# irfanfadhullah/unet_zoo

Measured on AMD Instinct MI355X. Metric: images/sec (fwd+bwd) at B=16 3x256x256, 1/2/4/8 MI355X, higher is better.
Workload: dtype bf16; 1 GPU; unet train step (zero_grad+fwd+BCE+bwd+clip+AdamW), B=16/GPU 3x256x256, random-init weights; global_batch=16, parallelism=dp1

## Files before the change

include/unetzoo_hip.h:

```cpp
#ifndef UNETZOO_HIP_H
#define UNETZOO_HIP_H

#include <stddef.h>
#include <stdint.h>

#ifdef __cplusplus
extern "C" {
#endif

#define UZ_ABI_VERSION 1

enum { UZ_F32 = 0, UZ_BF16 = 1 };

enum {
  UZ_OK = 0,
  UZ_EINVAL = -1,
  UZ_ENOTIMPL = -2
};

enum {
  UZ_TAPS_CONV = 0,
  UZ_TAPS_GATHER2X2 = 1,
  UZ_TAPS_CONV_UP2 = 2,
  UZ_TAPS_CONV_S2 = 3
// ... 5 lines not shown

int uz_abi_version(void);
const char* uz_last_error_string(void);
int uz_profile_arm(void* start_event, void* stop_event);
int uz_profile_disarm(void);
int uz_build_ablate(void);
const char* uz_source_hash(void);
int uz_clock_probe(int iters, void* out_pairs, int workgroups, void* stream);
int uz_set_cu_reserve(int n);
int uz_get_cu_reserve(void);

typedef struct uz_conv_desc {
  int dtype;
  int N, H, W;
  int Hin, Win;
  int Cin, ldx;
  int Nout, ldy;
  int ntaps, taps_mode, dil;
  int store_mode, Co;
  int Hout, Wout;
} uz_conv_desc;

int uz_conv_igemm_grid_m(const uz_conv_desc* d);
int uz_conv_igemm_kernel_name(const uz_conv_desc* d, int with_workspace, char* buf, int cap);
int uz_conv_igemm(const uz_conv_desc* d, const void* x, const void* w_packed, const float* bias,
                  void* y, float* stats_partial, void* stream);
int uz_conv_igemm_res(const uz_conv_desc* d, const void* x, const void* w_packed, const float* bias,
                      const void* res, int ldres, void* y, void* stream);
int uz_conv_igemm_res_ws(const uz_conv_desc* d, const void* x, const void* w_packed, const float* bias,
                         const void* res, int ldres, void* y, void* workspace, void* stream);
long long uz_conv_igemm_workspace_bytes(const uz_conv_desc* d);
int uz_conv_igemm_ws_grid_m(const uz_conv_desc* d);
int uz_conv_igemm_ws(const uz_conv_desc* d, const void* x, const void* w_packed, const float* bias,
                     void* y, float* stats_partial, void* workspace, void* stream);
int uz_conv_igemm_bnred_supported(const uz_conv_desc* d);
int uz_conv_igemm_bnred(const uz_conv_desc* d, const void* x, const void* w_packed, void* y, const void* bn_y,
                        int ld_bny, const float* scale, const float* shift, const float* mean, const float* invstd,
                        float* partial, void* stream);

int uz_conv_igemm_xf_supported(const uz_conv_desc* d);
int uz_conv_igemm_xf(const uz_conv_desc* d, const void* x, const float* in_scale, const float* in_shift,
                     const void* w_packed, const float* bias, void* y, float* stats_partial, void* stream);

typedef struct uz_wgrad_desc {
  int dtype;
  int N, H, W;
  int Hr, Wr;
  int Ci, ldl;
  int Cj, ldr;
  int ntaps, taps_mode, dil;
} uz_wgrad_desc;

int uz_wgrad_split(const uz_wgrad_desc* d);
long long uz_wgrad_workspace_bytes(const uz_wgrad_desc* d);
int uz_wgrad(const uz_wgrad_desc* d, const void* L, const void* R, float* out, void* workspace,
             void* stream);
int uz_wgrad_kernel_name(const uz_wgrad_desc* d, char* buf, int cap);
int uz_wgrad_xf_supported(const uz_wgrad_desc* d);
int uz_wgrad_xf(const uz_wgrad_desc* d, const void* L, const void* R, const float* r_scale, const float* r_shift,
                float* out, void* workspace, void* stream, int phase);
int uz_wgrad_phase(const uz_wgrad_desc* d, const void* L, const void* R, float* out, void* workspace, void* stream,
                   int phase);
typedef struct {
  uz_wgrad_desc desc;
  const void* L;
  const void* R;
  float* out;
} uz_wgrad_item;
long long uz_wgrad_multi_workspace_bytes(const uz_wgrad_item* items, int n);
int uz_wgrad_multi(const uz_wgrad_item* items, int n, void* workspace, void* stream);
long long uz_wgrad_batched_workspace_bytes(const uz_wgrad_desc* d, int batch);
int uz_wgrad_batched(const uz_wgrad_desc* d, int batch, const void* L, long long lb, const void* R, long long rb,
                     float* out, long long ob, void* workspace, void* stream);
int uz_wgrad_batched2(const uz_wgrad_desc* d, int batch, int batch2, const void* L, long long lb, long long lb2, const void* R,
                      long long rb, long long rb2, float* out, long long ob, void* workspace, void* stream);

int uz_conv3x3_first_supported(int dtype, int C, int Cout);
int uz_conv3x3_first_rows(int N, int H, int W);
int uz_conv3x3_first_fwd(int dtype, const float* x, int N, int C, int H, int W, const float* w, const float* bias, int Cout,
                         void* y, int ldy, float* stats, void* stream);
long long uz_conv3x3_first_wgrad_workspace_bytes(int N, int H, int W, int Cout);
int uz_conv3x3_first_wgrad(int dtype, const float* x, int N, int C, int H, int W, const void* dy, int lddy, int Cout, float* dw,
                           void* workspace, void* stream);

enum { UZ_PACK_CONV_FWD = 0, UZ_PACK_CONV_DGRAD = 1, UZ_PACK_CONVT_FWD = 2, UZ_PACK_CONVT_DGRAD = 3,
       UZ_PACK_IM2COL = 4, UZ_PACK_VEC_REPEAT = 5 };
int uz_pack_weights(int dtype, int mode, const float* w, int Co, int Ci, int T, int Kpad, void* dst,
                    void* stream);
typedef struct uz_pack_item {
  const float* src;
  void* dst;
  long long begin;
  int mode, Co, Ci, T, Kpad;
  int pad_;
} uz_pack_item;
int uz_pack_weights_batched(int dtype, const uz_pack_item* items_device, int n_items,
                            long long total_elements, void* stream);
typedef struct uz_pack3x3_item {
  const float* src;
  void* dst_fwd;
  void* dst_dgrad;
  int Co, Ci;
  int tile_begin;
  int pad_;
} uz_pack3x3_item;
int uz_pack_conv3x3_batched(int dtype, const uz_pack3x3_item* items_device, int n_items, int total_tiles,
                            void* stream);

int uz_im2col3x3_nchw(int dtype, const float* x_nchw, int N, int C, int H, int W, int Kpad, void* dst,
                      void* stream);

int uz_bn_finalize(const float* stats_partial, int grid_m, int C, double count, const float* gamma,
                   const float* beta, float eps, float momentum, float* running_mean,
                   float* running_var, float* scale, float* shift, float* mean, float* invstd,
                   void* stream);
int uz_bn_eval_scale(int C, const float* gamma, const float* beta, const float* running_mean,
                     const float* running_var, float eps, float* scale, float* shift, void* stream);

int uz_bn_relu_apply(int dtype, const void* y, int ldy, const float* scale, const float* shift,
                     int N, int H, int W, int C, void* act, int lda, void* pooled, int ldp,
                     void* stream);
int uz_bn_relu_add_apply(int dtype, const void* y, int ldy, const float* scale, const float* shift,
                         int N, int H, int W, int C, const void* res, int ldr, void* act, int lda,
                         void* pooled, int ldp, int pool_ceil, void* stream);
int uz_bn_relu_add_apply_fin(int dtype, const void* y, int ldy, const float* stats_partial, int rows, double count,
                             const float* gamma, const float* beta, float eps, float momentum, float* running_mean,
                             float* running_var, float* vec, int* flag, int N, int H, int W, int C, const void* res, int ldr,
                             void* act, int lda, void* pooled, int ldp, int pool_ceil, void* stream);

typedef struct uz_bnbwd_desc {
  int dtype;
  int N, H, W, C;
  int ldy, ldg0, ldg1, ldgp, lddy;
  int pool_ceil;
} uz_bnbwd_desc;
int uz_colstats_rows(int dtype, int P, int C);
int uz_colstats(int dtype, const void* x, int ld, int P, int C, float* partial, void* stream);
long long uz_bn_relu_bwd_workspace_bytes(const uz_bnbwd_desc* d, int has_pool_grad);
int uz_bn_relu_bwd_reduce(const uz_bnbwd_desc* d, const void* y, const float* scale,
                          const float* shift, const float* mean, const float* invstd, const void* g0,
                          const void* g1, const void* gpool, void* workspace, double* sums,
                          float* dgamma, float* dbeta, void* stream);
int uz_bn_relu_bwd_apply(const uz_bnbwd_desc* d, const void* y, const float* scale,
                         const float* shift, const float* mean, const float* invstd, const void* g0,
                         const void* g1, const void* gpool, const double* sums, double count,
                         void* dy, void* stream);
int uz_bn_relu_bwd_reduce_rows(const uz_bnbwd_desc* d, const void* y, const float* scale, const float* shift,
                               const float* mean, const float* invstd, const void* g0, const void* g1, const void* gpool,
                               void* workspace, void* stream);
int uz_bn_relu_bwd_apply_fin(const uz_bnbwd_desc* d, const void* y, const float* scale, const float* shift,
                             const float* mean, const float* invstd, const void* g0, const void* g1, const void* gpool,
                             const float* partial, int rows, double* sums, float* dgamma, float* dbeta, int* flag,
                             double count, void* dy, void* stream);
int uz_bn_bwd_finalize(const float* partial, int rows, int C, double* sums, float* dgamma, float* dbeta, void* stream);

int uz_outconv_fwd(int dtype, const void* x, int ldx, int N, int HW, int C, const float* w,
                   const float* b, int Kout, float* out_nchw, void* stream);
int uz_outconv_fwd_xf(int dtype, const void* y, int ldy, int N, int HW, int C, const float* scale, const float* shift,
                      const float* w, const float* b, int Kout, float* out_nchw, void* stream);
long long uz_outconv_bwd_workspace_bytes(int dtype, int N, int HW, int C, int Kout);
int uz_outconv_bwd(int dtype, const void* x, int ldx, int N, int HW, int C, const float* w, int Kout,
                   const float* g_nchw, void* dx, int lddx, float* dw, float* db, void* workspace,
                   void* stream);
int uz_outconv_bwd_rows(int dtype, int N, int HW, int C);
int uz_outconv_bwd_bnred(int dtype, const void* x, int ldx, int N, int HW, int C, const float* w, int Kout,
                         const float* g_nchw, void* dx, int lddx, float* dw, float* db, void* workspace,
                         const void* bn_y, int ld_bny, const float* scale, const float* shift, const float* mean,
                         const float* invstd, float* bn_partial, void* stream);

int uz_attn_grid(int dtype, int P, int channels);
int uz_attn_psi_fwd(int dtype, const void* g1raw, int ldg, const void* x1raw, int ldx, const float* vec_g,
                    const float* vec_x, const float* wpsi, const float* bpsi ,
                    int P, int F, float* q, float* partial , void* stream);
int uz_attn_gate_fwd(int dtype, const void* x, int ldx, const float* q, const float* vec_q, int P, int C,
                     void* out, int ldo, void* stream);
int uz_attn_bwd_psi(int dtype, const void* dout, int ldd, const void* x, int ldx, const float* q,
                    const float* vec_q, int P, int C, void* dx_direct, int lddx, float* dz,
                    float* partial , void* stream);
int uz_attn_bwd_reduce(int dtype, const void* g1raw, int ldg, const void* x1raw, int ldx, const float* q,
                       const float* dz, const float* wpsi, const float* vec_g, const float* vec_x,
                       const float* vec_q, const double* a01, int P, int F,
                       float* partial , void* stream);
int uz_attn_bwd_apply(int dtype, const void* g1raw, int ldg, const void* x1raw, int ldx, const float* q,
                      const float* dz, const float* wpsi, const float* vec_g, const float* vec_x,
                      const float* vec_q, const double* a01, const double* totals, int P, int F,
                      void* dg1raw, int lddg, void* dx1raw, int lddx, void* stream);
int uz_sum_rows(const float* partial, int rows, int n, double* out, void* stream);
int uz_sum_rows_f32(const float* partial, int rows, int n, float* out0, int n0, float* out1, void* stream);
int uz_sum_rows_f32_ld(const float* partial, int ld, int rows, int n, float* out0, int n0, float* out1,
                       void* stream);
int uz_sum2x2(int dtype, const void* du, int ldu, int N, int H, int W, int C, void* dx, int lddx,
              void* stream);

int uz_bilinear_fwd(int dtype, const void* x, int ldx, long long x_img_stride, int N, int Hi, int Wi,
                    int C, void* y, int ldy, long long y_img_stride, int Ho, int Wo, void* stream);
int uz_bilinear_bwd(int dtype, const void* g, int ldg, long long g_img_stride, int N, int Hi, int Wi,
                    int C, void* dx, int lddx, long long dx_img_stride, int Ho, int Wo, void* stream);
int uz_resize_bilinear_fwd(int dtype, const void* x, int ldx, long long x_img_stride, int N, int Hi, int Wi,
                           int C, void* y, int ldy, long long y_img_stride, int Ho, int Wo, int align_corners,
                           void* stream);
int uz_resize_bilinear_bwd(int dtype, const void* g, int ldg, long long g_img_stride, int N, int Hi, int Wi,
                           int C, void* dx, int lddx, long long dx_img_stride, int Ho, int Wo, int align_corners,
                           void* stream);
int uz_resample2(int dtype, const void* src, int lds, int N, int Hs, int Ws, int C, void* dst, int ldd, int Hd,
                 int Wd, int mode, void* stream);
int uz_pool_grad_combine(int dtype, int N, int H, int W, int C, const void* act, int lda, const void* g0,
                         int ldg0, const void* g1, int ldg1, const void* gp, int ldgp, void* out, int ldo,
                         int pool_ceil, void* stream);
int uz_sideconv3x3_fwd(int dtype, const void* x, int ldx, int N, int H, int W, int C, const float* w,
                       const float* bias, float* taps_ws, float* out, long long out_img_stride,
                       void* stream);
long long uz_sideconv3x3_bwd_workspace_bytes(int dtype, int N, int H, int W, int C);
int uz_sideconv3x3_bwd(int dtype, const void* x, int ldx, int N, int H, int W, int C, const float* w,
                       const float* g, long long g_img_stride, void* dx, int lddx, float* dw, float* db,
                       void* workspace, void* stream);
int uz_fuse1x1_fwd(const float* d, int N, int HW, int Cc, int K, const float* w, const float* b,
                   float* out, void* stream);
long long uz_fuse1x1_bwd_workspace_bytes(int N, int HW, int Cc, int K);
int uz_fuse1x1_bwd(const float* d, int N, int HW, int Cc, int K, const float* w, const float* g,
                   const float* const* g_extra, int n_extra, float* dcat, float* dw, float* db,
                   void* workspace, void* stream);

int uz_patchify(int dtype, const float* x_nchw, int N, int C, int H, int W, int patch, int Kpad,
                void* out, void* stream);

enum { UZ_LN_PLAIN = 0, UZ_LN_MERGE = 1, UZ_LN_EXPAND = 2 };
typedef struct uz_ln_desc {
  int dtype, N, Ho, Wo, C;
  int ldx, ldy, ldr, ldg, lddx;
  int mode, r;
  float eps;
  int act;
} uz_ln_desc;
int uz_layernorm_fwd(const uz_ln_desc* d, const void* x, const float* gamma, const float* beta,
                     const void* res, const float* image_scale, void* y, float* stats, void* stream);
int uz_layernorm_bwd_rows(const uz_ln_desc* d);
int uz_layernorm_bwd(const uz_ln_desc* d, const void* x, const float* gamma, const float* stats,
// ... 185 lines not shown
```

unet_zoo_amd/_lib.py:

```python
from __future__ import annotations

import ctypes
import os
from ctypes import POINTER, Structure, c_char_p, c_double, c_float, c_int, c_void_p

import torch

UZ_F32, UZ_BF16 = 0, 1
TAPS_CONV, TAPS_GATHER2X2, TAPS_CONV_UP2, TAPS_CONV_S2 = 0, 1, 2, 3
STORE_PLAIN, STORE_SHUFFLE2X2 = 0, 1
PACK_CONV_FWD, PACK_CONV_DGRAD, PACK_CONVT_FWD, PACK_CONVT_DGRAD, PACK_IM2COL, PACK_VEC_REPEAT = range(6)

LIB_NAME = "libunetzoo_hip.so"
LIB_PATH = os.environ.get("UNET_ZOO_AMD_LIB") or os.path.join(os.path.dirname(os.path.abspath(__file__)), LIB_NAME)

EXPORTS = (
    "uz_abi_version", "uz_last_error_string", "uz_build_ablate", "uz_source_hash", "uz_set_cu_reserve", "uz_get_cu_reserve", "uz_clock_probe", "uz_conv_igemm_grid_m", "uz_conv_igemm",
    "uz_wgrad_split", "uz_wgrad_workspace_bytes", "uz_wgrad", "uz_wgrad_kernel_name", "uz_wgrad_phase", "uz_wgrad_xf_supported", "uz_wgrad_xf", "uz_conv3x3_first_supported", "uz_conv3x3_first_rows", "uz_conv3x3_first_fwd",
    "uz_conv3x3_first_wgrad_workspace_bytes", "uz_conv3x3_first_wgrad", "uz_pack_weights", "uz_pack_weights_batched", "uz_pack_conv3x3_batched", "uz_im2col3x3_nchw", "uz_bn_finalize",
    "uz_bn_eval_scale", "uz_bn_relu_apply", "uz_bn_relu_bwd_workspace_bytes", "uz_bn_relu_bwd_reduce", "uz_bn_relu_bwd_apply",
    "uz_outconv_fwd", "uz_outconv_fwd_xf", "uz_outconv_bwd_workspace_bytes", "uz_outconv_bwd", "uz_outconv_bwd_rows", "uz_outconv_bwd_bnred",
    "uz_colsum",
    "uz_attn_grid", "uz_attn_psi_fwd", "uz_attn_gate_fwd", "uz_attn_bwd_psi", "uz_attn_bwd_reduce",
    "uz_attn_bwd_apply", "uz_sum_rows", "uz_sum_rows_f32", "uz_sum2x2",
    "uz_bn_relu_add_apply", "uz_bn_relu_add_apply_fin", "uz_bn_relu_bwd_reduce_rows", "uz_bn_relu_bwd_apply_fin", "uz_bilinear_fwd", "uz_bilinear_bwd", "uz_resize_bilinear_fwd", "uz_resize_bilinear_bwd", "uz_resample2",
    "uz_pool_grad_combine",
    "uz_sideconv3x3_fwd", "uz_sideconv3x3_bwd_workspace_bytes", "uz_sideconv3x3_bwd",
    "uz_fuse1x1_fwd", "uz_fuse1x1_bwd_workspace_bytes", "uz_fuse1x1_bwd",
    "uz_conv_igemm_workspace_bytes", "uz_conv_igemm_ws_grid_m", "uz_conv_igemm_ws",
    "uz_conv_igemm_bnred_supported", "uz_conv_igemm_bnred", "uz_conv_igemm_xf_supported", "uz_conv_igemm_xf", "uz_conv_igemm_kernel_name", "uz_bn_bwd_finalize", "uz_profile_arm", "uz_profile_disarm",
    "uz_patchify", "uz_layernorm_fwd", "uz_layernorm_bwd_rows", "uz_layernorm_bwd", "uz_layernorm_act_bwd",
    "uz_ln_head_fwd", "uz_ln_head_bwd_workspace_bytes", "uz_ln_head_bwd", "uz_sum_rows_f32_ld",
    "uz_winattn_fwd", "uz_winattn_bwd_rows", "uz_winattn_bwd",
    "uz_colsum_workspace_bytes", "uz_colsum_ws", "uz_colstats_rows", "uz_colstats", "uz_cpb_fwd", "uz_cpb_bwd",
    "uz_cpb_fwd_batched", "uz_cpb_bwd_batched_workspace_bytes", "uz_cpb_bwd_batched",
    "uz_clip_adamw_workspace_bytes", "uz_clip_adamw",
    "uz_gelu_fwd", "uz_gelu_bwd", "uz_dwconv3x3", "uz_dwconv3x3_wgrad_rows", "uz_dwconv3x3_wgrad",
    "uz_space_to_depth", "uz_space_to_depth_crop", "uz_im2col_nchw", "uz_sra_fwd", "uz_sra_bwd_workspace_bytes", "uz_sra_bwd",
    "uz_bce_dice_workspace_bytes", "uz_bce_dice", "uz_colsum_batched_workspace_bytes", "uz_colsum_batched", "uz_sum_rows_f32_batched", "uz_conv_igemm_res", "uz_wgrad_multi_workspace_bytes", "uz_wgrad_multi", "uz_conv_igemm_res_ws",
    "uz_add_relu", "uz_relu_bwd", "uz_pil_resample_h_u8", "uz_pil_resample_v_f32",
    "uz_gemm_nt", "uz_softmax_fwd", "uz_softmax_bwd", "uz_adaptive_avgpool_fwd", "uz_adaptive_avgpool_bwd",
    "uz_rowdot_f32", "uz_cast_rows", "uz_wgrad_batched_workspace_bytes", "uz_wgrad_batched", "uz_wgrad_batched2",
    "uz_softmax_workspace_bytes", "uz_add_map", "uz_dropout", "uz_chanscale_relu", "uz_chanattn_probs_fwd", "uz_chanattn_probs_bwd",
    "uz_conv5x5_grid_m", "uz_conv5x5", "uz_wgrad5x5_workspace_bytes", "uz_wgrad5x5",
    "uz_bn_elu_apply", "uz_bn_elu_bwd_rows", "uz_bn_elu_bwd_reduce", "uz_bn_elu_bwd_apply",
)


class ConvDesc(Structure):
    _fields_ = [(n, c_int) for n in (
        "dtype", "N", "H", "W", "Hin", "Win", "Cin", "ldx", "Nout", "ldy", "ntaps", "taps_mode",
        "dil", "store_mode", "Co", "Hout", "Wout")]


class WgradDesc(Structure):
    _fields_ = [(n, c_int) for n in (
        "dtype", "N", "H", "W", "Hr", "Wr", "Ci", "ldl", "Cj", "ldr", "ntaps", "taps_mode", "dil")]


class Conv5Desc(Structure):
    _fields_ = [(n, c_int) for n in ("dtype", "N", "H", "W", "Cin", "ldx", "Nout", "ldy", "ksize")]


class Wgrad5Desc(Structure):
    _fields_ = [(n, c_int) for n in ("dtype", "N", "H", "W", "Ci", "ldl", "Cj", "ldr", "ksize", "CiOut", "CjOut")]


class BnEluBwdDesc(Structure):
    _fields_ = [(n, c_int) for n in ("dtype", "N", "HW", "C", "ldx", "ldo", "ldg0", "ldg1", "ldg2", "lddx", "ldgres", "flags")]


class BnBwdDesc(Structure):
    _fields_ = [(n, c_int) for n in (
        "dtype", "N", "H", "W", "C", "ldy", "ldg0", "ldg1", "ldgp", "lddy", "pool_ceil")]


class LnDesc(Structure):
    _fields_ = [(n, c_int) for n in ("dtype", "N", "Ho", "Wo", "C", "ldx", "ldy", "ldr", "ldg", "lddx", "mode", "r")] \
        + [("eps", c_float), ("act", c_int)]


class WinAttnDesc(Structure):
    _fields_ = [(n, c_int) for n in ("dtype", "B", "H", "W", "C", "heads", "ws", "shift", "Nt", "ldq", "ldo")] \
        + [("scale", c_float)]


class SraDesc(Structure):
    _fields_ = [(n, c_int) for n in ("dtype", "B", "N", "NK", "heads", "head_dim", "kps", "ldq", "ldk", "ldv", "ldo")] \
        + [("scale", c_float)]


class GemmDesc(Structure):
    _fields_ = [(n, c_int) for n in ("dtype", "batch", "M", "N", "K", "ldx", "ldw", "ldy", "ldres")] \
        + [(n, ctypes.c_longlong) for n in ("xb", "wb", "yb", "resb")] + [("batch2", c_int)] \
        + [(n, ctypes.c_longlong) for n in ("xb2", "wb2", "yb2", "resb2")]


class WgradItem(Structure):
    _fields_ = [("desc", WgradDesc), ("L", c_void_p), ("R", c_void_p), ("out", c_void_p)]


class SumRowsItem(Structure):
    _fields_ = [("partial", c_void_p), ("out0", c_void_p), ("out1", c_void_p), ("rows", c_int), ("n", c_int), ("n0", c_int),
                ("reserved", c_int)]
# ... 16 lines not shown
    _fields_ = [("src", c_void_p), ("dst", c_void_p), ("begin", ctypes.c_longlong), ("mode", c_int),
                ("Co", c_int), ("Ci", c_int), ("T", c_int), ("Kpad", c_int), ("pad_", c_int)]


class Pack3x3Item(Structure):
    _fields_ = [("src", c_void_p), ("dst_fwd", c_void_p), ("dst_dgrad", c_void_p), ("Co", c_int), ("Ci", c_int),
                ("tile_begin", c_int), ("pad_", c_int)]


class HipLibraryError(RuntimeError):
    pass


_lib = None


def load():
    global _lib
    if _lib is not None:
        return _lib
    if not os.path.exists(LIB_PATH):
        raise HipLibraryError(
            f"{LIB_PATH} not found: the HIP kernel library is not built. Run "
            "`python -c 'import __graft_entry__ as g; g.build()'` from the repo root. "
            "unet_zoo_amd has no CPU fallback.")
    lib = ctypes.CDLL(LIB_PATH)
    lib.uz_abi_version.restype = c_int
    lib.uz_last_error_string.restype = c_char_p
    lib.uz_source_hash.restype = c_char_p
    lib.uz_source_hash.argtypes = []
    vp, ip, fp = c_void_p, c_int, c_float
    lib.uz_set_cu_reserve.argtypes = [c_int]
    lib.uz_clock_probe.argtypes = [c_int, vp, c_int, vp]
    lib.uz_get_cu_reserve.argtypes = []
    lib.uz_conv_igemm_grid_m.argtypes = [POINTER(ConvDesc)]
    lib.uz_conv_igemm.argtypes = [POINTER(ConvDesc), vp, vp, vp, vp, vp, vp]
    lib.uz_conv_igemm_res.argtypes = [POINTER(ConvDesc), vp, vp, vp, vp, ip, vp, vp]
    lib.uz_conv_igemm_res_ws.argtypes = [POINTER(ConvDesc), vp, vp, vp, vp, ip, vp, vp, vp]
    lib.uz_conv_igemm_workspace_bytes.argtypes = [POINTER(ConvDesc)]
    lib.uz_conv_igemm_ws_grid_m.argtypes = [POINTER(ConvDesc)]
    lib.uz_conv_igemm_ws.argtypes = [POINTER(ConvDesc), vp, vp, vp, vp, vp, vp, vp]
    lib.uz_conv_igemm_bnred_supported.argtypes = [POINTER(ConvDesc)]
    lib.uz_conv_igemm_xf_supported.argtypes = [POINTER(ConvDesc)]
    lib.uz_conv_igemm_xf.argtypes = [POINTER(ConvDesc), vp, vp, vp, vp, vp, vp, vp, vp]
    lib.uz_conv_igemm_kernel_name.argtypes = [POINTER(ConvDesc), c_int, c_char_p, c_int]
    lib.uz_profile_arm.argtypes = [vp, vp]
    lib.uz_profile_disarm.argtypes = []
    lib.uz_conv_igemm_bnred.argtypes = [POINTER(ConvDesc), vp, vp, vp, vp, c_int, vp, vp, vp, vp, vp, vp]
    lib.uz_bn_bwd_finalize.argtypes = [vp, c_int, c_int, vp, vp, vp, vp]
    lib.uz_patchify.argtypes = [ip, vp, ip, ip, ip, ip, ip, ip, vp, vp]
    lib.uz_layernorm_fwd.argtypes = [POINTER(LnDesc), vp, vp, vp, vp, vp, vp, vp, vp]
    lib.uz_layernorm_act_bwd.argtypes = [POINTER(LnDesc), vp, vp, vp, vp, vp, vp, vp, vp]
    lib.uz_layernorm_bwd_rows.argtypes = [POINTER(LnDesc)]
    lib.uz_layernorm_bwd.argtypes = [POINTER(LnDesc), vp, vp, vp, vp, vp, vp, vp, vp]
    lib.uz_ln_head_fwd.argtypes = [POINTER(LnDesc), vp, vp, vp, vp, vp, ip, vp, vp, vp]
    lib.uz_ln_head_bwd_workspace_bytes.argtypes = [POINTER(LnDesc), ip]
    lib.uz_ln_head_bwd.argtypes = [POINTER(LnDesc), vp, vp, vp, vp, ip, vp, vp, vp, vp, vp, vp, vp, vp, vp]
    lib.uz_sum_rows_f32_ld.argtypes = [vp, ip, ip, ip, vp, ip, vp, vp]
    lib.uz_winattn_fwd.argtypes = [POINTER(WinAttnDesc), vp, vp, vp, vp, vp, vp]
    lib.uz_winattn_bwd_rows.argtypes = [POINTER(WinAttnDesc)]
    lib.uz_winattn_bwd.argtypes = [POINTER(WinAttnDesc), vp, vp, vp, vp, vp, vp, ip, vp, ip, vp, vp]
    lib.uz_colstats_rows.argtypes = [ip, ip, ip]
    lib.uz_colstats.argtypes = [ip, vp, ip, ip, ip, vp, vp]
    lib.uz_cpb_fwd.argtypes = [vp, vp, vp, vp, vp, ip, ip, ip, vp, vp]
    lib.uz_cpb_bwd.argtypes = [vp, vp, vp, vp, vp, ip, ip, ip, vp, vp, vp, vp, vp]
    lib.uz_cpb_fwd_batched.argtypes = [vp, ip, vp]
    lib.uz_cpb_bwd_batched_workspace_bytes.argtypes = [vp, ip]
    lib.uz_cpb_bwd_batched.argtypes = [vp, ip, vp, vp]
    lib.uz_clip_adamw_workspace_bytes.argtypes = []
    lib.uz_clip_adamw.argtypes = [vp, vp, vp, vp, ctypes.c_longlong, fp, fp, fp, fp, fp, fp, vp, vp, vp]
    lib.uz_wgrad_split.argtypes = [POINTER(WgradDesc)]
    lib.uz_wgrad_workspace_bytes.argtypes = [POINTER(WgradDesc)]
    lib.uz_wgrad.argtypes = [POINTER(WgradDesc), vp, vp, vp, vp, vp]
    lib.uz_wgrad_kernel_name.argtypes = [POINTER(WgradDesc), c_char_p, c_int]
    lib.uz_wgrad_phase.argtypes = [POINTER(WgradDesc), vp, vp, vp, vp, vp, c_int]
    lib.uz_wgrad_xf_supported.argtypes = [POINTER(WgradDesc)]
    lib.uz_wgrad_xf.argtypes = [POINTER(WgradDesc), vp, vp, vp, vp, vp, vp, vp, c_int]
    lib.uz_conv3x3_first_supported.argtypes = [ip, ip, ip]
    lib.uz_conv3x3_first_rows.argtypes = [ip, ip, ip]
    lib.uz_conv3x3_first_fwd.argtypes = [ip, vp, ip, ip, ip, ip, vp, vp, ip, vp, ip, vp, vp]
    lib.uz_conv3x3_first_wgrad_workspace_bytes.argtypes = [ip, ip, ip, ip]
    lib.uz_conv3x3_first_wgrad_workspace_bytes.restype = ctypes.c_longlong
    lib.uz_conv3x3_first_wgrad.argtypes = [ip, vp, ip, ip, ip, ip, vp, ip, ip, vp, vp, vp]
    lib.uz_pack_weights.argtypes = [ip, ip, vp, ip, ip, ip, ip, vp, vp]
    lib.uz_pack_weights_batched.argtypes = [ip, vp, ip, ctypes.c_longlong, vp]
    lib.uz_pack_conv3x3_batched.argtypes = [ip, vp, ip, ip, vp]
    lib.uz_im2col3x3_nchw.argtypes = [ip, vp, ip, ip, ip, ip, ip, vp, vp]
    lib.uz_bn_finalize.argtypes = [vp, ip, ip, c_double, vp, vp, fp, fp, vp, vp, vp, vp, vp, vp, vp]
    lib.uz_bn_eval_scale.argtypes = [ip, vp, vp, vp, vp, fp, vp, vp, vp]
    lib.uz_bn_relu_apply.argtypes = [ip, vp, ip, vp, vp, ip, ip, ip, ip, vp, ip, vp, ip, vp]
    lib.uz_bn_relu_bwd_workspace_bytes.argtypes = [POINTER(BnBwdDesc), ip]
    lib.uz_bn_relu_bwd_reduce.argtypes = [POINTER(BnBwdDesc), vp, vp, vp, vp, vp, vp, vp, vp, vp, vp,
                                          vp, vp, vp]
    lib.uz_bn_relu_bwd_apply.argtypes = [POINTER(BnBwdDesc), vp, vp, vp, vp, vp, vp, vp, vp, vp,
                                         c_double, vp, vp]
    lib.uz_outconv_fwd.argtypes = [ip, vp, ip, ip, ip, ip, vp, vp, ip, vp, vp]
    lib.uz_outconv_fwd_xf.argtypes = [ip, vp, ip, ip, ip, ip, vp, vp, vp, vp, ip, vp, vp]
    lib.uz_outconv_bwd_workspace_bytes.argtypes = [ip, ip, ip, ip, ip]
    lib.uz_outconv_bwd.argtypes = [ip, vp, ip, ip, ip, ip, vp, ip, vp, vp, ip, vp, vp, vp, vp]
    lib.uz_outconv_bwd_rows.argtypes = [ip, ip, ip, ip]
    lib.uz_outconv_bwd_bnred.argtypes = [ip, vp, ip, ip, ip, ip, vp, ip, vp, vp, ip, vp, vp, vp, vp, ip, vp, vp, vp, vp, vp, vp]
    lib.uz_colsum.argtypes = [ip, vp, ip, ip, ip, vp, vp]
    lib.uz_colsum_workspace_bytes.argtypes = [ip, ip, ip]
    lib.uz_colsum_ws.argtypes = [ip, vp, ip, ip, ip, vp, vp, vp]
    lib.uz_attn_grid.argtypes = [ip, ip, ip]
    lib.uz_attn_psi_fwd.argtypes = [ip, vp, ip, vp, ip, vp, vp, vp, vp, ip, ip, vp, vp, vp]
    lib.uz_attn_gate_fwd.argtypes = [ip, vp, ip, vp, vp, ip, ip, vp, ip, vp]
    lib.uz_attn_bwd_psi.argtypes = [ip, vp, ip, vp, ip, vp, vp, ip, ip, vp, ip, vp, vp, vp]
    lib.uz_attn_bwd_reduce.argtypes = [ip, vp, ip, vp, ip, vp, vp, vp, vp, vp, vp, vp, ip, ip, vp, vp]
    lib.uz_attn_bwd_apply.argtypes = [ip, vp, ip, vp, ip, vp, vp, vp, vp, vp, vp, vp, vp, ip, ip, vp, ip,
                                      vp, ip, vp]
    lib.uz_sum_rows.argtypes = [vp, ip, ip, vp, vp]
    lib.uz_sum_rows_f32.argtypes = [vp, ip, ip, vp, ip, vp, vp]
    lib.uz_sum2x2.argtypes = [ip, vp, ip, ip, ip, ip, ip, vp, ip, vp]
    ll = ctypes.c_longlong
    lib.uz_bn_relu_add_apply.argtypes = [ip, vp, ip, vp, vp, ip, ip, ip, ip, vp, ip, vp, ip, vp, ip, ip, vp]
    lib.uz_bn_relu_add_apply_fin.argtypes = [ip, vp, ip, vp, ip, ctypes.c_double, vp, vp, c_float, c_float, vp, vp, vp, vp,
                                             ip, ip, ip, ip, vp, ip, vp, ip, vp, ip, ip, vp]
    lib.uz_bn_relu_bwd_reduce_rows.argtypes = [POINTER(BnBwdDesc), vp, vp, vp, vp, vp, vp, vp, vp, vp, vp]
    lib.uz_bn_relu_bwd_apply_fin.argtypes = [POINTER(BnBwdDesc), vp, vp, vp, vp, vp, vp, vp, vp, vp, ip, vp, vp, vp, vp,
                                             ctypes.c_double, vp, vp]
    lib.uz_bilinear_fwd.argtypes = [ip, vp, ip, ll, ip, ip, ip, ip, vp, ip, ll, ip, ip, vp]
    lib.uz_bilinear_bwd.argtypes = [ip, vp, ip, ll, ip, ip, ip, ip, vp, ip, ll, ip, ip, vp]
    lib.uz_resize_bilinear_fwd.argtypes = [ip, vp, ip, ll, ip, ip, ip, ip, vp, ip, ll, ip, ip, ip, vp]
    lib.uz_resize_bilinear_bwd.argtypes = [ip, vp, ip, ll, ip, ip, ip, ip, vp, ip, ll, ip, ip, ip, vp]
    lib.uz_resample2.argtypes = [ip, vp, ip, ip, ip, ip, ip, vp, ip, ip, ip, ip, vp]
    lib.uz_pool_grad_combine.argtypes = [ip, ip, ip, ip, ip, vp, ip, vp, ip, vp, ip, vp, ip, vp, ip, ip, vp]
    lib.uz_sideconv3x3_fwd.argtypes = [ip, vp, ip, ip, ip, ip, ip, vp, vp, vp, vp, ll, vp]
    lib.uz_sideconv3x3_bwd_workspace_bytes.argtypes = [ip, ip, ip, ip, ip]
    lib.uz_sideconv3x3_bwd.argtypes = [ip, vp, ip, ip, ip, ip, ip, vp, vp, ll, vp, ip, vp, vp, vp, vp]
    lib.uz_fuse1x1_fwd.argtypes = [vp, ip, ip, ip, ip, vp, vp, vp, vp]
    lib.uz_fuse1x1_bwd_workspace_bytes.argtypes = [ip, ip, ip, ip]
    lib.uz_fuse1x1_bwd.argtypes = [vp, ip, ip, ip, ip, vp, vp, POINTER(c_void_p), ip, vp, vp, vp, vp, vp]
    lib.uz_sum_rows_f32_batched.argtypes = [POINTER(SumRowsItem), ip, vp]
    lib.uz_wgrad_multi_workspace_bytes.argtypes = [POINTER(WgradItem), ip]
    lib.uz_wgrad_multi_workspace_bytes.restype = ctypes.c_longlong
    lib.uz_wgrad_multi.argtypes = [POINTER(WgradItem), ip, vp, vp]
    lib.uz_colsum_batched_workspace_bytes.argtypes = [ip, POINTER(ColsumItem), ip]
    lib.uz_colsum_batched.argtypes = [ip, POINTER(ColsumItem), ip, vp, vp]
    lib.uz_bce_dice_workspace_bytes.argtypes = [ll]
    lib.uz_bce_dice.argtypes = [vp, vp, ll, vp, vp, vp, vp]
    lib.uz_gelu_fwd.argtypes = [ip, vp, ip, vp, ip, ll, ip, vp]
    lib.uz_gelu_bwd.argtypes = [ip, vp, ip, vp, ip, vp, ip, ll, ip, vp]
    lib.uz_dwconv3x3.argtypes = [ip, vp, ip, vp, vp, vp, ip, ip, ip, ip, ip, ip, vp]
    lib.uz_dwconv3x3_wgrad_rows.argtypes = [ip, ip, ip, ip, ip]
    lib.uz_dwconv3x3_wgrad.argtypes = [ip, vp, ip, vp, ip, vp, ip, ip, ip, ip, vp]
    lib.uz_space_to_depth.argtypes = [ip, vp, ip, vp, ip, ip, ip, ip, ip, ip, ip, vp]
    lib.uz_space_to_depth_crop.argtypes = [ip, vp, ip, vp, ip, ip, ip, ip, ip, ip, ip, vp]
    lib.uz_im2col_nchw.argtypes = [ip, vp, ip, ip, ip, ip, ip, ip, ip, ip, vp, vp]
    lib.uz_sra_fwd.argtypes = [POINTER(SraDesc), vp, vp, vp, vp, vp, vp]
    lib.uz_sra_bwd_workspace_bytes.argtypes = [POINTER(SraDesc)]
    lib.uz_sra_bwd.argtypes = [POINTER(SraDesc), vp, vp, vp, vp, vp, vp, ip, vp, ip, vp, ip, vp, vp]
    lib.uz_add_relu.argtypes = [ip, vp, ip, vp, ip, vp, ip, ll, ip, vp]
    lib.uz_relu_bwd.argtypes = [ip, vp, ip, vp, ip, vp, ip, ll, ip, vp]
    lib.uz_pil_resample_h_u8.argtypes = [vp, ip, ip, ip, vp, vp, ip, ip, vp, vp]
    lib.uz_pil_resample_v_f32.argtypes = [vp, ip, ip, ip, vp, vp, ip, ip, POINTER(c_float), POINTER(c_float), ip, vp, vp]
    lib.uz_wgrad_batched_workspace_bytes.argtypes = [POINTER(WgradDesc), ip]
    lib.uz_wgrad_batched.argtypes = [POINTER(WgradDesc), ip, vp, ll, vp, ll, vp, ll, vp, vp]
    lib.uz_wgrad_batched2.argtypes = [POINTER(WgradDesc), ip, ip, vp, ll, ll, vp, ll, ll, vp, ll, vp, vp]
    lib.uz_gemm_nt.argtypes = [POINTER(GemmDesc), vp, vp, vp, vp, vp, vp]
    lib.uz_softmax_workspace_bytes.argtypes = [ip, ip, ip, ip]
    lib.uz_softmax_fwd.argtypes = [ip, vp, ip, ll, ip, ip, ip, ip, c_float, vp, vp]
    lib.uz_chanattn_probs_fwd.argtypes = [ip, vp, ip, ip, ip, ip, c_float, c_float, vp, vp, vp]
    lib.uz_chanattn_probs_bwd.argtypes = [ip, vp, vp, ip, ip, ip, ip, c_float, c_float, vp, vp, vp]
    lib.uz_dropout.argtypes = [ip, vp, ip, vp, c_float, vp, ip, ll, ip, vp]
    lib.uz_chanscale_relu.argtypes = [ip, ip, vp, ip, vp, ip, vp, vp, ip, ip, ip, vp, ip, vp]
    lib.uz_add_map.argtypes = [ip, vp, ip, vp, vp, ip, ll, ip, ip, vp]
    lib.uz_softmax_bwd.argtypes = [ip, vp, vp, ip, ll, ip, ip, ip, ip, c_float, vp, ip, vp]
    lib.uz_adaptive_avgpool_fwd.argtypes = [ip, vp, ip, ip, ip, ip, ip, vp, ip, ip, ip, vp]
    lib.uz_adaptive_avgpool_bwd.argtypes = [ip, vp, ip, ip, ip, ip, ip, vp, ip, ip, ip, ip, vp]
    lib.uz_rowdot_f32.argtypes = [ip, vp, ip, vp, ip, ll, ip, vp, vp]
    lib.uz_cast_rows.argtypes = [ip, vp, ip, vp, ip, ll, ip, ip, vp]
    lib.uz_conv5x5_grid_m.argtypes = [POINTER(Conv5Desc)]
    lib.uz_conv5x5.argtypes = [POINTER(Conv5Desc), vp, vp, vp, vp, vp, vp]
    lib.uz_wgrad5x5_workspace_bytes.argtypes = [POINTER(Wgrad5Desc)]
    lib.uz_wgrad5x5.argtypes = [POINTER(Wgrad5Desc), vp, vp, vp, vp, vp]
    lib.uz_bn_elu_apply.argtypes = [ip, vp, ip, vp, vp, ip, ip, ip, vp, ip, vp, ip, vp, ip, vp, ip, vp]
    lib.uz_bn_elu_bwd_rows.argtypes = [POINTER(BnEluBwdDesc)]
    lib.uz_bn_elu_bwd_reduce.argtypes = [POINTER(BnEluBwdDesc), vp, vp, vp, vp, vp, vp, vp, vp, vp, vp, vp, vp]
    lib.uz_bn_elu_bwd_apply.argtypes = [POINTER(BnEluBwdDesc), vp, vp, vp, vp, vp, vp, vp, vp, vp, vp, vp, vp, vp, vp]
    for name in EXPORTS:
        fn = getattr(lib, name)
        if name not in ("uz_last_error_string", "uz_source_hash"):
# ... 74 lines not shown
```

unet_zoo_amd/csrc/uz_conv_first.hip:

```cpp
#include "uz_common.h"

namespace {

constexpr int TH = 8, TW = 32, PH = TH + 2, PW = TW + 2;
constexpr int STG = 144;

struct CfArgs {
  const float* x;
  const float* w;
  const float* bias;
  void* y;
  float* stats;
  const void* dy;
  float* slab;
  int N, C, H, W, Cout, ldy, th_n, tw_n, ntiles;
};

__device__ __forceinline__ float round_bf16(float v) { return (float)(bf16_t)v; }

__device__ __forceinline__ unsigned halo_fetch(const CfArgs& a, float (&h)[4], int tile, int tid) {
  const int per = a.th_n * a.tw_n;
  const int img = tile / per, rem = tile - img * per;
  const int h0 = (rem / a.tw_n) * TH, w0 = (rem % a.tw_n) * TW;
  const int n = a.C * PH * PW;
  unsigned mask = 0;
#pragma unroll
  for (int j = 0; j < 4; ++j) {
    const int idx = tid + 256 * j;
    const int c = idx / (PH * PW), r2 = idx - c * (PH * PW);
    const int r = r2 / PW, col = r2 - r * PW;
    const int gh = h0 - 1 + r, gw = w0 - 1 + col;
    const bool ok = idx < n && (unsigned)gh < (unsigned)a.H && (unsigned)gw < (unsigned)a.W;
    h[j] = a.x[ok ? (((size_t)img * a.C + c) * a.H + gh) * a.W + gw : 0];
    mask |= ok ? 1u << j : 0u;
  }
  return mask;
}
__device__ __forceinline__ void halo_store(float* sx, const float (&h)[4], unsigned mask, int tid, int n) {
#pragma unroll
  for (int j = 0; j < 4; ++j)
    if (tid + 256 * j < n) sx[tid + 256 * j] = (mask >> j & 1u) ? round_bf16(h[j]) : 0.f;
}
static_assert(3 * PH * PW <= 4 * 256, "four halo elements per thread");

template <int CT>
__global__ __launch_bounds__(256) void conv_first_fwd_kernel(const CfArgs a) {
  __shared__ float sx[3 * PH * PW];
  __shared__ __attribute__((aligned(16))) float sbias[64];
  __shared__ __attribute__((aligned(16))) char sstg[4][32 * STG];
  __shared__ float sred[4][2][CT * 32];
  const int tid = threadIdx.x, lane = tid & 63, wave = tid >> 6;
  const int px = lane & 31, b = lane >> 5;
  const int per = a.th_n * a.tw_n;
  const int K = a.C * 9;
  float hreg[4];
  unsigned hmask = 0;
  if ((int)blockIdx.x < a.ntiles) hmask = halo_fetch(a, hreg, blockIdx.x, tid);
  if (tid < 64) sbias[tid] = (a.bias != nullptr && tid < a.Cout) ? a.bias[tid] : 0.f;

  bf16x8 wfr[CT][2];
  float wraw[CT][2][8];
#pragma unroll
  for (int t = 0; t < CT; ++t)
#pragma unroll
    for (int kh = 0; kh < 2; ++kh)
#pragma unroll
      for (int i = 0; i < 8; ++i) {
        const int k = 16 * kh + 8 * b + i, co = 32 * t + px;
        wraw[t][kh][i] = a.w[(k < K && co < a.Cout) ? (size_t)co * K + k : 0];
      }
#pragma unroll
  for (int t = 0; t < CT; ++t)
#pragma unroll
    for (int kh = 0; kh < 2; ++kh)
#pragma unroll
      for (int i = 0; i < 8; ++i) asm volatile("" : "+v"(wraw[t][kh][i]));
#pragma unroll
  for (int t = 0; t < CT; ++t)
#pragma unroll
    for (int kh = 0; kh < 2; ++kh)
#pragma unroll
      for (int i = 0; i < 8; ++i) {
        const int k = 16 * kh + 8 * b + i, co = 32 * t + px;
        wfr[t][kh][i] = (bf16_t)((k < K && co < a.Cout) ? wraw[t][kh][i] : 0.f);
      }
  int koff[2][8];
#pragma unroll
  for (int kh = 0; kh < 2; ++kh)
#pragma unroll
    for (int i = 0; i < 8; ++i) {
      const int k = 16 * kh + 8 * b + i;
      const int c = k / 9, t9 = k - c * 9, ty = t9 / 3, tx = t9 - ty * 3;
      koff[kh][i] = (k < K ? (c * PH + ty) * PW + tx : 0) + px;
    }
  constexpr int CPP = CT * 4;
  constexpr int PPI = 64 / CPP;
  const int ch = lane % CPP;
  float st1[8], st2[8];
// ... 1 lines not shown
  for (int e = 0; e < 8; ++e) st1[e] = st2[e] = 0.f;

  char* stg = sstg[wave];
  bf16_t* yg = static_cast<bf16_t*>(a.y);
#pragma unroll 1
  for (int tile = blockIdx.x; tile < a.ntiles; tile += gridDim.x) {
    const int img = tile / per, rem = tile - img * per;
    const int h0 = (rem / a.tw_n) * TH, w0 = (rem % a.tw_n) * TW;
    __syncthreads();
    halo_store(sx, hreg, hmask, tid, a.C * PH * PW);
    __syncthreads();
    {
      const int nxt = tile + (int)gridDim.x;
      hmask = halo_fetch(a, hreg, nxt < a.ntiles ? nxt : tile, tid);
    }
#pragma unroll
    for (int rr = 0; rr < 2; ++rr) {
      const int row = 2 * wave + rr, gh = h0 + row;
      bf16x8 pfr[2];
#pragma unroll
      for (int kh = 0; kh < 2; ++kh)
#pragma unroll
        for (int i = 0; i < 8; ++i) pfr[kh][i] = (bf16_t)sx[koff[kh][i] + row * PW];
#pragma unroll
      for (int t = 0; t < CT; ++t) {
        f32x16 acc;
#pragma unroll
        for (int r = 0; r < 16; ++r) acc[r] = 0.f;
        acc = __builtin_amdgcn_mfma_f32_32x32x16_bf16(wfr[t][0], pfr[0], acc, 0, 0, 0);
        acc = __builtin_amdgcn_mfma_f32_32x32x16_bf16(wfr[t][1], pfr[1], acc, 0, 0, 0);
#pragma unroll
        for (int g4 = 0; g4 < 4; ++g4) {
          const f32x4 bq = *reinterpret_cast<const f32x4*>(sbias + 32 * t + 8 * g4 + 4 * b);
          bf16x4 o;
#pragma unroll
          for (int e = 0; e < 4; ++e) o[e] = (bf16_t)(acc[4 * g4 + e] + bq[e]);
          *reinterpret_cast<bf16x4*>(stg + px * STG + (32 * t + 8 * g4 + 4 * b) * 2) = o;
        }
      }
      __builtin_amdgcn_wave_barrier();
#pragma unroll
      for (int j = 0; j < 32 / PPI; ++j) {
        const int p = j * PPI + lane / CPP;
        const bf16x8 v = *reinterpret_cast<const bf16x8*>(stg + p * STG + ch * 16);
        const int gw = w0 + p;
        if (gh < a.H && gw < a.W && ch * 8 < a.Cout) {
          *reinterpret_cast<bf16x8*>(yg + (((size_t)img * a.H + gh) * a.W + gw) * a.ldy + ch * 8) = v;
#pragma unroll
          for (int e = 0; e < 8; ++e) {
            const float f = (float)v[e];
            st1[e] += f;
            st2[e] += f * f;
          }
        }
      }
      __builtin_amdgcn_wave_barrier();
    }
  }
  if (a.stats == nullptr) return;
  __syncthreads();
  float* red = reinterpret_cast<float*>(sstg[wave]);
#pragma unroll
  for (int e = 0; e < 8; ++e) {
    red[lane * 16 + e] = st1[e];
    red[lane * 16 + 8 + e] = st2[e];
  }
  __builtin_amdgcn_wave_barrier();
#pragma unroll
  for (int idx = lane; idx < CPP * 16; idx += 64) {
    const int c2 = idx / 16, v2 = idx % 16;
    float sacc = 0.f;
#pragma unroll
    for (int q = 0; q < PPI; ++q) sacc += red[(q * CPP + c2) * 16 + v2];
    sred[wave][v2 >> 3][c2 * 8 + (v2 & 7)] = sacc;
  }
  __syncthreads();
  if (tid < 2 * CT * 32) {
    const int q = tid / (CT * 32), co = tid % (CT * 32);
    const float sum = (sred[0][q][co] + sred[1][q][co]) + (sred[2][q][co] + sred[3][q][co]);
    if (co < a.Cout) a.stats[((size_t)blockIdx.x * 2 + q) * a.Cout + co] = sum;
  }
}

template <int CT>
__global__ __launch_bounds__(256) void conv_first_wgrad_kernel(const CfArgs a) {
  constexpr int RB = CT * 64;
  __shared__ float sx[3 * PH * PW];
  __shared__ __attribute__((aligned(16))) char sdy[TH * TW * RB];
  static_assert(4 * CT * 16 * 64 * 4 == TH * TW * RB, "the waves' accumulators meet in the dy tile's LDS");
  float (*sacc)[CT][16][64] = reinterpret_cast<float (*)[CT][16][64]>(sdy);
  const int tid = threadIdx.x, lane = tid & 63, wave = tid >> 6;
  const int l31 = lane & 31, b = lane >> 5;
  const int per = a.th_n * a.tw_n;
  const int K = a.C * 9;
  const bf16_t* dyg = static_cast<const bf16_t*>(a.dy);

  const int k = l31;
  const int kc = k / 9, kt = k - kc * 9, kty = kt / 3, ktx = kt - kty * 3;
  const int pbase = (k < K) ? (kc * PH + kty) * PW + ktx + 8 * b : 0;
  const int g = lane >> 4, q4 = (lane & 15) >> 2, p4 = lane & 3;
  const int lk = 8 * (g >> 1) + q4, lcol = 16 * (g & 1) + 4 * p4;
  typedef __attribute__((address_space(3))) bf16x4* lds_bf16x4_ptr;

  f32x16 acc[CT];
#pragma unroll
  for (int t = 0; t < CT; ++t)
#pragma unroll
    for (int r = 0; r < 16; ++r) acc[t][r] = 0.f;

  constexpr int CPP = RB / 16;
  constexpr int NDY = TH * TW * CPP / 256;
  float hreg[4];
  f32x4 dreg[NDY];
  unsigned hmask = 0, dmask = 0;
  auto dy_fetch = [&](int tile) __attribute__((always_inline)) {
    const int img = tile / per, rem = tile - img * per;
    const int h0 = (rem / a.tw_n) * TH, w0 = (rem % a.tw_n) * TW;
#pragma unroll
    for (int j = 0; j < NDY; ++j) {
      const int idx = tid + 256 * j;
      const int p = idx / CPP, ch = idx % CPP;
      const int r = p / TW, c = p % TW, gh = h0 + r, gw = w0 + c;
      const bool ok = gh < a.H && gw < a.W && ch * 8 < a.Cout;
      dreg[j] = *reinterpret_cast<const f32x4*>(ok ? dyg + (((size_t)img * a.H + gh) * a.W + gw) * a.ldy + ch * 8 : dyg);
      dmask |= ok ? 1u << j : 0u;
    }
  };
  if ((int)blockIdx.x < a.ntiles) {
    hmask = halo_fetch(a, hreg, blockIdx.x, tid);
    dy_fetch(blockIdx.x);
  }
#pragma unroll 1
  for (int tile = blockIdx.x; tile < a.ntiles; tile += gridDim.x) {
    __syncthreads();
    halo_store(sx, hreg, hmask, tid, a.C * PH * PW);
#pragma unroll
    for (int j = 0; j < NDY; ++j) {
      const int idx = tid + 256 * j;
      const int p = idx / CPP, ch = idx % CPP;
      const int gran = ch >> 2, sw = (p >> 1) & 1;
      const int pg = (CT == 2) ? (gran ^ sw) : gran;
      const f32x4 z4 = {0.f, 0.f, 0.f, 0.f};
      *reinterpret_cast<f32x4*>(sdy + p * RB + pg * 64 + (ch & 3) * 16) = (dmask >> j & 1u) ? dreg[j] : z4;
    }
    __syncthreads();
    {
      const int nxt = tile + (int)gridDim.x, ft = nxt < a.ntiles ? nxt : tile;
      hmask = halo_fetch(a, hreg, ft, tid);
      dmask = 0;
      dy_fetch(ft);
    }
#pragma unroll
    for (int rr = 0; rr < 2; ++rr)
#pragma unroll
      for (int half = 0; half < 2; ++half) {
        const int row = 2 * wave + rr, c0 = 16 * half;
        bf16x8 pfr;
#pragma unroll
        for (int i = 0; i < 8; ++i) pfr[i] = (bf16_t)sx[pbase + row * PW + c0 + i];
#pragma unroll
        for (int t = 0; t < CT; ++t) {
          const int p = row * TW + c0 + lk;
          const int sw = (p >> 1) & 1;
          const int gr = (CT == 2) ? (t ^ sw) : 0;
          const char* ad = sdy + p * RB + gr * 64 + lcol * 2;
          const bf16x4 lo = __builtin_amdgcn_ds_read_tr16_b64_v4bf16((lds_bf16x4_ptr)(ad));
          const bf16x4 hi = __builtin_amdgcn_ds_read_tr16_b64_v4bf16((lds_bf16x4_ptr)(ad + 4 * RB));
          const bf16x8 dfr = __builtin_shufflevector(lo, hi, 0, 1, 2, 3, 4, 5, 6, 7);
          acc[t] = __builtin_amdgcn_mfma_f32_32x32x16_bf16(dfr, pfr, acc[t], 0, 0, 0);
        }
      }
  }
  __syncthreads();
#pragma unroll
  for (int t = 0; t < CT; ++t)
#pragma unroll
    for (int r = 0; r < 16; ++r) sacc[wave][t][r][lane] = acc[t][r];
  __syncthreads();
  for (int idx = tid; idx < CT * 16 * 64; idx += 256) {
    const int t = idx / (16 * 64), r = (idx / 64) % 16, l = idx % 64;
    const float s = (sacc[0][t][r][l] + sacc[1][t][r][l]) + (sacc[2][t][r][l] + sacc[3][t][r][l]);
    const int co = 32 * t + (r & 3) + 8 * (r >> 2) + 4 * (l >> 5), kk = l & 31;
    if (co < a.Cout) a.slab[((size_t)blockIdx.x * a.Cout + co) * 32 + kk] = s;
  }
}

__global__ __launch_bounds__(256) void conv_first_wgrad_reduce_kernel(const float* __restrict__ slab, int nwg, int Cout, int K,
                                                                     float* __restrict__ dw) {
  __shared__ float part[16][17];
  const int o = threadIdx.x & 15, zg = threadIdx.x >> 4;
  const int idx = blockIdx.x * 16 + o;
  const size_t stride = (size_t)Cout * 32;
  float s = 0.f;
  int z = zg;
  for (; z + 7 * 16 < nwg; z += 8 * 16) {
    float v[8];
#pragma unroll
    for (int u = 0; u < 8; ++u) v[u] = slab[(size_t)(z + 16 * u) * stride + idx];
#pragma unroll
    for (int u = 0; u < 8; ++u) s += v[u];
  }
  for (; z < nwg; z += 16) s += slab[(size_t)z * stride + idx];
  part[zg][o] = s;
  __syncthreads();
  if (zg == 0) {
    float t = 0.f;
#pragma unroll
    for (int q = 0; q < 16; ++q) t += part[q][o];
    const int co = idx >> 5, k = idx & 31;
    if (k < K) dw[(size_t)co * K + k] = t;
  }
}

int check(int dtype, int N, int C, int H, int W, int Cout, int ld, const char* what) {
  UZ_REQUIRE(dtype == UZ_BF16, "%s: bf16 only (the fp32 run mode takes the im2col path)", what);
  UZ_REQUIRE(N > 0 && H > 0 && W > 0 && C >= 1 && C <= 3, "%s: C = %d not in 1 .. 3", what, C);
  UZ_REQUIRE((Cout == 32 || Cout == 64) && ld >= Cout && ld % 8 == 0, "%s: Cout = %d (32 or 64), ld = %d", what, Cout, ld);
  UZ_REQUIRE((long long)N * H * W * ld * 2 < (1LL << 40), "%s: too large", what);
  return UZ_OK;
}

void fill(CfArgs& a, int N, int C, int H, int W, int Cout, int ld) {
  a.N = N;
  a.C = C;
  a.H = H;
  a.W = W;
  a.Cout = Cout;
  a.ldy = ld;
  a.th_n = (H + TH - 1) / TH;
  a.tw_n = (W + TW - 1) / TW;
  a.ntiles = N * a.th_n * a.tw_n;
}

}

extern "C" int uz_conv3x3_first_supported(int dtype, int C, int Cout) {
  return dtype == UZ_BF16 && C >= 1 && C <= 3 && (Cout == 32 || Cout == 64);
}

static int first_fwd_grid(int ntiles) {
  const int cap = 3 * UZ_NUM_CU_HW;
  return ntiles < cap ? ntiles : cap;
}

extern "C" int uz_conv3x3_first_rows(int N, int H, int W) {
  return first_fwd_grid(N * ((H + TH - 1) / TH) * ((W + TW - 1) / TW));
}

extern "C" int uz_conv3x3_first_fwd(int dtype, const float* x, int N, int C, int H, int W, const float* w, const float* bias,
                                    int Cout, void* y, int ldy, float* stats, void* stream) {
  const int rc = check(dtype, N, C, H, W, Cout, ldy, "uz_conv3x3_first_fwd");
  if (rc != UZ_OK) return rc;
  UZ_REQUIRE(x && w && y && ((uintptr_t)y & 15) == 0, "uz_conv3x3_first_fwd: null / unaligned pointer");
  CfArgs a = {};
  a.x = x;
  a.w = w;
  a.bias = bias;
  a.y = y;
  a.stats = stats;
  fill(a, N, C, H, W, Cout, ldy);
  hipStream_t s = static_cast<hipStream_t>(stream);
  const int grid = first_fwd_grid(a.ntiles);
  if (Cout == 64) hipLaunchKernelGGL(conv_first_fwd_kernel<2>, dim3(grid), dim3(256), 0, s, a);
  else hipLaunchKernelGGL(conv_first_fwd_kernel<1>, dim3(grid), dim3(256), 0, s, a);
  UZ_LAUNCH_CHECK("uz_conv3x3_first_fwd");
  return UZ_OK;
}

static int first_wgrad_grid(int ntiles) {
  const int cap = 3 * UZ_NUM_CU_HW;
  return ntiles < cap ? ntiles : cap;
}

extern "C" long long uz_conv3x3_first_wgrad_workspace_bytes(int N, int H, int W, int Cout) {
  const int ntiles = N * ((H + TH - 1) / TH) * ((W + TW - 1) / TW);
  return (long long)first_wgrad_grid(ntiles) * Cout * 32 * (long long)sizeof(float);
}

extern "C" int uz_conv3x3_first_wgrad(int dtype, const float* x, int N, int C, int H, int W, const void* dy, int lddy,
                                      int Cout, float* dw, void* workspace, void* stream) {
  const int rc = check(dtype, N, C, H, W, Cout, lddy, "uz_conv3x3_first_wgrad");
  if (rc != UZ_OK) return rc;
  UZ_REQUIRE(x && dy && dw && workspace && ((uintptr_t)dy & 15) == 0, "uz_conv3x3_first_wgrad: null / unaligned pointer");
  CfArgs a = {};
  a.x = x;
  a.dy = dy;
  a.slab = static_cast<float*>(workspace);
  fill(a, N, C, H, W, Cout, lddy);
  const int grid = first_wgrad_grid(a.ntiles);
  hipStream_t s = static_cast<hipStream_t>(stream);
  if (Cout == 64) hipLaunchKernelGGL(conv_first_wgrad_kernel<2>, dim3(grid), dim3(256), 0, s, a);
  else hipLaunchKernelGGL(conv_first_wgrad_kernel<1>, dim3(grid), dim3(256), 0, s, a);
  UZ_LAUNCH_CHECK("uz_conv3x3_first_wgrad");
  hipLaunchKernelGGL(conv_first_wgrad_reduce_kernel, dim3(Cout * 32 / 16), dim3(256), 0, s, a.slab, grid, Cout, C * 9, dw);
  UZ_LAUNCH_CHECK("uz_conv3x3_first_wgrad(reduce)");
  return UZ_OK;
}
```

unet_zoo_amd/csrc/uz_eltwise.hip:

```cpp
#include "uz_common.h"

namespace {

template <typename T> __device__ __forceinline__ void load_f(const T* p, float* f) {
  const Vec16<T> v = ld16(p);
#pragma unroll
  for (int i = 0; i < ElemTraits<T>::VEC; ++i) f[i] = (float)v.v[i];
}
template <typename T> __device__ __forceinline__ void store_f(T* p, const float* f) {
  Vec16<T> v;
#pragma unroll
  for (int i = 0; i < ElemTraits<T>::VEC; ++i) v.v[i] = (T)f[i];
  st16(p, v);
}

template <int EW>
__global__ __launch_bounds__(1024) void bn_finalize_kernel(
    const float* __restrict__ part, int grid_m, int C, double count, const float* __restrict__ gamma,
    const float* __restrict__ beta, float eps, float momentum, float* running_mean,
    float* running_var, float* scale, float* shift, float* mean, float* invstd) {
  constexpr int NG = 1024 / EW;
  __shared__ double sh[2][NG][EW + 1];
  const int cl = threadIdx.x % EW, g = threadIdx.x / EW;
  const int c = blockIdx.x * EW + cl;
// ... 414 lines not shown
        for (int i = 0; i < VEC; ++i) yv[k][i] = gv[k][i] = 0.f;
        continue;
      }
      load_f(y + p * a.ldy + c0, yv[k]);
      if (g0 != nullptr) {
        load_f(g0 + p * a.ldg0 + c0, gv[k]);
      } else {
#pragma unroll
        for (int i = 0; i < VEC; ++i) gv[k][i] = 0.f;
      }
      if (g1 != nullptr) {
        float t[VEC];
        load_f(g1 + p * a.ldg1 + c0, t);
#pragma unroll
        for (int i = 0; i < VEC; ++i) gv[k][i] += t[i];
      }
    }
#endif
    if constexpr (POOL) {
      if (gp != nullptr && has_pool) {
        float gpv[VEC];
#ifndef UZ_BN_BRANCHY
#pragma unroll
        for (int i = 0; i < VEC; ++i) gpv[i] = (float)gpr.v[i];
#else
        load_f(gp + gpoff + c0, gpv);
#endif
#pragma unroll
        for (int i = 0; i < VEC; ++i) {
          float best = fmaf(yv[0][i], sc[i], sh[i]);
          if (!norelu) best = fmaxf(best, 0.f);
          int bk = 0;
#pragma unroll
          for (int k = 1; k < 4; ++k) {
            float v = fmaf(yv[k][i], sc[i], sh[i]);
            if (!norelu) v = fmaxf(v, 0.f);
            if (in[k] && v > best) {
              best = v;
              bk = k;
            }
          }
#pragma unroll
          for (int k = 0; k < 4; ++k) gv[k][i] += (k == bk) ? gpv[i] : 0.f;
        }
      }
    }
#pragma unroll
    for (int k = 0; k < NPIX; ++k) {
      if (!in[k]) continue;
      float out[VEC];
#pragma unroll
      for (int i = 0; i < VEC; ++i) {
        const float pre = fmaf(yv[k][i], sc[i], sh[i]);
        const float dz = (norelu || pre > 0.f) ? gv[k][i] : 0.f;
        const float xh = (yv[k][i] - mu[i]) * is[i];
        if (PASS == 1) {
          S0[i] += dz;
          S1[i] += dz * xh;
        } else {
          out[i] = sc[i] * (dz - k0[i] - xh * k1[i]);
        }
      }
      if (PASS == 2) {
        store_f(dy + pix[k] * a.lddy + c0, out);
      }
    }
  }

  if (PASS == 1) {
    float* mine = red + ((size_t)threadIdx.y * blockDim.x + threadIdx.x) * (2 * VEC);
#pragma unroll
    for (int i = 0; i < VEC; ++i) {
      mine[i] = S0[i];
      mine[VEC + i] = S1[i];
    }
    __syncthreads();
    for (int e = threadIdx.y; e < 2 * VEC; e += blockDim.y) {
      float t = 0.f;
      for (int r = 0; r < (int)blockDim.y; ++r) t += red[((size_t)r * blockDim.x + threadIdx.x) * (2 * VEC) + e];
      if (cok) {
        const int which = e / VEC, ch = c0 + (e % VEC);
        a.partials[((size_t)blockIdx.x * 2 + which) * a.C + ch] = t;
      }
    }
  }
}

template <int EW>
__global__ __launch_bounds__(1024) void bn_bwd_finalize_kernel(const float* __restrict__ part, int rows,
                                                               int C, double* __restrict__ sums,
                                                               float* dgamma, float* dbeta) {
  constexpr int NG = 1024 / EW;
  __shared__ double sh[2][NG][EW + 1];
  const int cl = threadIdx.x % EW, g = threadIdx.x / EW;
  const int c = blockIdx.x * EW + cl;
  double a1 = 0.0, a2 = 0.0;
  const int cq = c < C ? c : 0;
  for (int r = g; r < rows; r += 4 * NG) {
    float p1[4], p2[4];
#pragma unroll
    for (int k = 0; k < 4; ++k) {
      const int rr = r + k * NG < rows ? r + k * NG : 0;
      p1[k] = part[((size_t)rr * 2 + 0) * C + cq];
      p2[k] = part[((size_t)rr * 2 + 1) * C + cq];
    }
#pragma unroll
    for (int k = 0; k < 4; ++k) asm volatile("" : "+v"(p1[k]), "+v"(p2[k]));
#pragma unroll
    for (int k = 0; k < 4; ++k)
      if (r + k * NG < rows && c < C) {
        a1 += (double)p1[k];
        a2 += (double)p2[k];
      }
  }
  sh[0][g][cl] = a1;
  sh[1][g][cl] = a2;
  __syncthreads();
#pragma unroll
  for (int st = NG / 2; st > 0; st >>= 1) {
    if (g < st) {
      sh[0][g][cl] += sh[0][g + st][cl];
      sh[1][g][cl] += sh[1][g + st][cl];
    }
    __syncthreads();
  }
  if (g == 0 && c < C) {
    const double t1 = sh[0][0][cl], t2 = sh[1][0][cl];
    sums[c] = t1;
    sums[C + c] = t2;
    if (dgamma != nullptr) {
      dbeta[c] = (float)t1;
      dgamma[c] = (float)t2;
    }
  }
}

constexpr int OUTCONV_MAXK = 8;
__host__ __device__ inline int lanes_per_pixel(int chunks) {
  int l = 1;
  while (l < chunks) l <<= 1;
  return l;
}

template <typename T, int KOUT, bool XF = false>
__global__ __launch_bounds__(256) void outconv_fwd_kernel(const T* __restrict__ x, int ldx, int N,
                                                          int HW, int C, const float* __restrict__ w,
                                                          const float* __restrict__ b,
                                                          float* __restrict__ out,
                                                          const float* __restrict__ xf_scale = nullptr,
                                                          const float* __restrict__ xf_shift = nullptr) {
  constexpr int VEC = ElemTraits<T>::VEC;
  const int LPP = lanes_per_pixel(C / VEC);
  const int ppb = blockDim.x / LPP;
  const int sub = threadIdx.x % LPP, pl = threadIdx.x / LPP;
  const bool live = sub < C / VEC;
  const int P = N * HW;
  float wr[KOUT][VEC];
#pragma unroll
  for (int k = 0; k < KOUT; ++k)
#pragma unroll
    for (int i = 0; i < VEC; ++i) wr[k][i] = live ? w[k * C + sub * VEC + i] : 0.f;
  float xsc[VEC], xsh[VEC];
  if constexpr (XF) {
#pragma unroll
    for (int i = 0; i < VEC; ++i) {
      xsc[i] = live ? xf_scale[sub * VEC + i] : 0.f;
// ... 815 lines not shown
  BnBwdArgs a = bnbwd_args(d, y, scale, shift, mean, invstd, g0, g1, gpool);
  a.partials = static_cast<float*>(workspace);
  hipStream_t s = (hipStream_t)stream;
  const int rc2 = d->dtype == UZ_BF16 ? bnbwd_launch<bf16_t, 1>(d, a, gpool != nullptr, s)
                                      : bnbwd_launch<float, 1>(d, a, gpool != nullptr, s);
  if (rc2 != UZ_OK) return rc2;
  dim3 grid, block;
  bnbwd_shape(d, gpool != nullptr, &grid, &block);
  bnbwd_finalize(static_cast<const float*>(workspace), (int)grid.x, d->C, sums, dgamma, dbeta, s);
  UZ_LAUNCH_CHECK("uz_bn_relu_bwd_reduce(finalize)");
  return UZ_OK;
}

extern "C" int uz_bn_bwd_finalize(const float* partial, int rows, int C, double* sums, float* dgamma, float* dbeta,
                                  void* stream) {
  UZ_REQUIRE(partial && sums && rows > 0 && C > 0, "uz_bn_bwd_finalize: bad arguments");
  UZ_REQUIRE((dgamma == nullptr) == (dbeta == nullptr), "uz_bn_bwd_finalize: dgamma/dbeta");
  bnbwd_finalize(partial, rows, C, sums, dgamma, dbeta, (hipStream_t)stream);
  UZ_LAUNCH_CHECK("uz_bn_bwd_finalize");
  return UZ_OK;
}

extern "C" int uz_bn_relu_bwd_apply(const uz_bnbwd_desc* d, const void* y, const float* scale,
                                    const float* shift, const float* mean, const float* invstd,
                                    const void* g0, const void* g1, const void* gpool, const double* sums,
                                    double count, void* dy, void* stream) {
  const int rc = bnbwd_check(d, g0, g1, gpool);
  if (rc != UZ_OK) return rc;
  UZ_REQUIRE(y && scale && shift && mean && invstd && sums && dy, "uz_bn_relu_bwd_apply: null pointer");
  UZ_REQUIRE(count > 0, "uz_bn_relu_bwd_apply: count");
  const int vec = d->dtype == UZ_BF16 ? 8 : 4;
  UZ_REQUIRE(d->lddy % vec == 0 && d->lddy >= d->C, "uz_bn_relu_bwd_apply: bad lddy");
  BnBwdArgs a = bnbwd_args(d, y, scale, shift, mean, invstd, g0, g1, gpool);
  a.sums = const_cast<double*>(sums);
  a.dy = dy;
  a.inv_count = 1.0 / count;
  hipStream_t s = (hipStream_t)stream;
  return d->dtype == UZ_BF16 ? bnbwd_launch<bf16_t, 2>(d, a, gpool != nullptr, s)
                             : bnbwd_launch<float, 2>(d, a, gpool != nullptr, s);
}

extern "C" int uz_bn_relu_bwd_reduce_rows(const uz_bnbwd_desc* d, const void* y, const float* scale, const float* shift,
                                          const float* mean, const float* invstd, const void* g0, const void* g1,
                                          const void* gpool, void* workspace, void* stream) {
  const int rc = bnbwd_check(d, g0, g1, gpool);
  if (rc != UZ_OK) return rc;
  UZ_REQUIRE(y && scale && shift && mean && invstd && workspace, "uz_bn_relu_bwd_reduce_rows: null pointer");
  BnBwdArgs a = bnbwd_args(d, y, scale, shift, mean, invstd, g0, g1, gpool);
  a.partials = static_cast<float*>(workspace);
  hipStream_t s = (hipStream_t)stream;
  return d->dtype == UZ_BF16 ? bnbwd_launch<bf16_t, 1>(d, a, gpool != nullptr, s) : bnbwd_launch<float, 1>(d, a, gpool != nullptr, s);
}

extern "C" int uz_bn_relu_bwd_apply_fin(const uz_bnbwd_desc* d, const void* y, const float* scale, const float* shift,
                                        const float* mean, const float* invstd, const void* g0, const void* g1,
                                        const void* gpool, const float* partial, int rows, double* sums, float* dgamma,
                                        float* dbeta, int* flag, double count, void* dy, void* stream) {
  const int rc = bnbwd_check(d, g0, g1, gpool);
  if (rc != UZ_OK) return rc;
  UZ_REQUIRE(y && scale && shift && mean && invstd && sums && dy && partial && flag, "uz_bn_relu_bwd_apply_fin: null pointer");
  UZ_REQUIRE(count > 0 && rows > 0, "uz_bn_relu_bwd_apply_fin: count / rows");
  UZ_REQUIRE((dgamma == nullptr) == (dbeta == nullptr), "uz_bn_relu_bwd_apply_fin: dgamma/dbeta");
  const int vec = d->dtype == UZ_BF16 ? 8 : 4;
  UZ_REQUIRE(d->lddy % vec == 0 && d->lddy >= d->C, "uz_bn_relu_bwd_apply_fin: bad lddy");
  BnBwdArgs a = bnbwd_args(d, y, scale, shift, mean, invstd, g0, g1, gpool);
  a.sums = sums;
  a.dy = dy;
  a.inv_count = 1.0 / count;
  a.fin.part = partial; a.fin.rows = rows; a.fin.ew = fin_ew(rows, d->C);
  a.fin.sums = sums; a.fin.dgamma = dgamma; a.fin.dbeta = dbeta; a.fin.flag = flag;
  hipStream_t s = (hipStream_t)stream;
  dim3 grid, block;
  bnbwd_shape(d, gpool != nullptr, &grid, &block, 2);
  if ((long long)grid.x * grid.y < (d->C + a.fin.ew - 1) / a.fin.ew) {
    bnbwd_finalize(partial, rows, d->C, sums, dgamma, dbeta, s);
    UZ_LAUNCH_CHECK("uz_bn_relu_bwd_apply_fin(finalize)");
    a.fin = BnFin{};
    return d->dtype == UZ_BF16 ? bnbwd_launch<bf16_t, 2>(d, a, gpool != nullptr, s) : bnbwd_launch<float, 2>(d, a, gpool != nullptr, s);
  }
  return d->dtype == UZ_BF16 ? bnbwd_launch<bf16_t, 2, true>(d, a, gpool != nullptr, s)
                             : bnbwd_launch<float, 2, true>(d, a, gpool != nullptr, s);
}

extern "C" int uz_outconv_fwd(int dtype, const void* x, int ldx, int N, int HW, int C, const float* w,
                              const float* b, int Kout, float* out_nchw, void* stream) {
  UZ_REQUIRE(dtype == UZ_F32 || dtype == UZ_BF16, "uz_outconv_fwd: bad dtype");
  const int vec = dtype == UZ_BF16 ? 8 : 4;
  UZ_REQUIRE(x && w && b && out_nchw, "uz_outconv_fwd: null pointer");
  UZ_REQUIRE(Kout >= 1 && Kout <= OUTCONV_MAXK, "uz_outconv_fwd: Kout=%d (max %d)", Kout, OUTCONV_MAXK);
  UZ_REQUIRE(C % vec == 0 && C / vec <= 64, "uz_outconv_fwd: C=%d unsupported", C);
  UZ_REQUIRE(ldx % vec == 0 && ldx >= C && N > 0 && HW > 0 && (long long)N * HW < (1LL << 31),
             "uz_outconv_fwd: bad shape");
  const int ppb = 256 / lanes_per_pixel(C / vec);
  const int grid = grid_for(((long long)N * HW + ppb - 1) / ppb, 1);
  hipStream_t s = (hipStream_t)stream;
  if (dtype == UZ_BF16) {
    UZ_KOUT_SWITCH(Kout, hipLaunchKernelGGL((outconv_fwd_kernel<bf16_t, KOUT>), dim3(grid), dim3(256), 0, s, (const bf16_t*)x, ldx, N, HW, C, w, b, out_nchw, (const float*)nullptr, (const float*)nullptr))
  } else {
    UZ_KOUT_SWITCH(Kout, hipLaunchKernelGGL((outconv_fwd_kernel<float, KOUT>), dim3(grid), dim3(256), 0, s, (const float*)x, ldx, N, HW, C, w, b, out_nchw, (const float*)nullptr, (const float*)nullptr))
  }
  UZ_LAUNCH_CHECK("uz_outconv_fwd");
  return UZ_OK;
}

extern "C" int uz_outconv_fwd_xf(int dtype, const void* y, int ldy, int N, int HW, int C, const float* scale,
                                 const float* shift, const float* w, const float* b, int Kout, float* out_nchw,
                                 void* stream) {
  UZ_REQUIRE(dtype == UZ_BF16, "uz_outconv_fwd_xf: bf16 only");
  UZ_REQUIRE(y && scale && shift && w && b && out_nchw, "uz_outconv_fwd_xf: null pointer");
  UZ_REQUIRE(Kout >= 1 && Kout <= OUTCONV_MAXK, "uz_outconv_fwd_xf: Kout=%d (max %d)", Kout, OUTCONV_MAXK);
  UZ_REQUIRE(C % 8 == 0 && C / 8 <= 64, "uz_outconv_fwd_xf: C=%d unsupported", C);
  UZ_REQUIRE(ldy % 8 == 0 && ldy >= C && N > 0 && HW > 0 && (long long)N * HW < (1LL << 31), "uz_outconv_fwd_xf: bad shape");
  const int ppb = 256 / lanes_per_pixel(C / 8);
  const int grid = grid_for(((long long)N * HW + ppb - 1) / ppb, 1);
  hipStream_t s = (hipStream_t)stream;
  UZ_KOUT_SWITCH(Kout, hipLaunchKernelGGL((outconv_fwd_kernel<bf16_t, KOUT, true>), dim3(grid), dim3(256), 0, s, (const bf16_t*)y, ldy, N, HW, C, w, b, out_nchw, scale, shift))
  UZ_LAUNCH_CHECK("uz_outconv_fwd_xf");
  return UZ_OK;
}

static int outconv_bwd_grid(int dtype, int N, int HW, int C) {
  const int vec = dtype == UZ_BF16 ? 8 : 4;
  const int ppb = 256 / lanes_per_pixel(C / vec);
  long long g = ((long long)N * HW + (long long)ppb * 4 - 1) / ((long long)ppb * 4);
  if (g > UZ_NUM_CU * 4) g = UZ_NUM_CU * 4;
  if (g < 1) g = 1;
  return (int)g;
}

extern "C" long long uz_outconv_bwd_workspace_bytes(int dtype, int N, int HW, int C, int Kout) {
  UZ_REQUIRE(dtype == UZ_F32 || dtype == UZ_BF16, "uz_outconv_bwd_workspace_bytes: bad dtype");
  const int vec = dtype == UZ_BF16 ? 8 : 4;
  UZ_REQUIRE(N > 0 && HW > 0 && Kout >= 1 && Kout <= OUTCONV_MAXK && C % vec == 0 && C / vec <= 64,
             "uz_outconv_bwd_workspace_bytes: bad shape");
  return (long long)outconv_bwd_grid(dtype, N, HW, C) * Kout * (C + 1) * (long long)sizeof(float);
}

extern "C" int uz_outconv_bwd_rows(int dtype, int N, int HW, int C) {
  UZ_REQUIRE(dtype == UZ_F32 || dtype == UZ_BF16, "uz_outconv_bwd_rows: bad dtype");
  return outconv_bwd_grid(dtype, N, HW, C);
}

extern "C" int uz_outconv_bwd_bnred(int dtype, const void* x, int ldx, int N, int HW, int C, const float* w,
                                    int Kout, const float* g_nchw, void* dx, int lddx, float* dw, float* db,
                                    void* workspace, const void* bn_y, int ld_bny, const float* scale,
                                    const float* shift, const float* mean, const float* invstd, float* bn_partial,
                                    void* stream) {
  UZ_REQUIRE(dtype == UZ_BF16, "uz_outconv_bwd_bnred: bf16 only");
  UZ_REQUIRE(w && g_nchw && dw && db && workspace && dx && bn_y && scale && shift && mean && invstd && bn_partial,
             "uz_outconv_bwd_bnred: null pointer");
  UZ_REQUIRE(Kout >= 1 && Kout <= OUTCONV_MAXK, "uz_outconv_bwd_bnred: Kout=%d", Kout);
  UZ_REQUIRE(C % 8 == 0 && C / 8 <= 64, "uz_outconv_bwd_bnred: C=%d unsupported", C);
  UZ_REQUIRE((x == nullptr || (ldx % 8 == 0 && ldx >= C)) && lddx % 8 == 0 && lddx >= C && ld_bny % 8 == 0 && ld_bny >= C && N > 0 &&
                 HW > 0 && (long long)N * HW < (1LL << 31), "uz_outconv_bwd_bnred: bad shape");
  const int g = outconv_bwd_grid(dtype, N, HW, C);
  float* part = static_cast<float*>(workspace);
  hipStream_t s = (hipStream_t)stream;
  if (x != nullptr) {
    UZ_KOUT_SWITCH(Kout, hipLaunchKernelGGL((outconv_bwd_kernel<bf16_t, KOUT, true>), dim3((unsigned)g), dim3(256), 0, s,
                                            (const bf16_t*)x, ldx, N, HW, C, w, g_nchw, (bf16_t*)dx, lddx, part,
                                            (const bf16_t*)bn_y, ld_bny, scale, shift, mean, invstd, bn_partial))
  } else {
    UZ_KOUT_SWITCH(Kout, hipLaunchKernelGGL((outconv_bwd_kernel<bf16_t, KOUT, true, true>), dim3((unsigned)g), dim3(256), 0, s,
                                            (const bf16_t*)nullptr, 0, N, HW, C, w, g_nchw, (bf16_t*)dx, lddx, part,
                                            (const bf16_t*)bn_y, ld_bny, scale, shift, mean, invstd, bn_partial))
  }
  UZ_LAUNCH_CHECK("uz_outconv_bwd_bnred");
  const int ne = Kout * (C + 1);
  hipLaunchKernelGGL(outconv_bwd_finalize_kernel, dim3(uz_cdiv(ne, 32)), dim3(1024), 0, s, part, g, Kout, C, dw, db);
  UZ_LAUNCH_CHECK("uz_outconv_bwd_bnred(finalize)");
  return UZ_OK;
}

extern "C" int uz_outconv_bwd(int dtype, const void* x, int ldx, int N, int HW, int C, const float* w,
                              int Kout, const float* g_nchw, void* dx, int lddx, float* dw, float* db,
                              void* workspace, void* stream) {
  UZ_REQUIRE(dtype == UZ_F32 || dtype == UZ_BF16, "uz_outconv_bwd: bad dtype");
  const int vec = dtype == UZ_BF16 ? 8 : 4;
  UZ_REQUIRE(x && w && g_nchw && dw && db && workspace, "uz_outconv_bwd: null pointer");
  UZ_REQUIRE(Kout >= 1 && Kout <= OUTCONV_MAXK, "uz_outconv_bwd: Kout=%d", Kout);
  UZ_REQUIRE(C % vec == 0 && C / vec <= 64, "uz_outconv_bwd: C=%d unsupported", C);
  UZ_REQUIRE(ldx % vec == 0 && ldx >= C && N > 0 && HW > 0 && (long long)N * HW < (1LL << 31),
             "uz_outconv_bwd: bad shape");
  if (dx) UZ_REQUIRE(lddx % vec == 0 && lddx >= C, "uz_outconv_bwd: bad lddx");
  const int g = outconv_bwd_grid(dtype, N, HW, C);
  float* part = static_cast<float*>(workspace);
  hipStream_t s = (hipStream_t)stream;
  if (dtype == UZ_BF16) {
    UZ_KOUT_SWITCH(Kout, hipLaunchKernelGGL((outconv_bwd_kernel<bf16_t, KOUT>), dim3((unsigned)g), dim3(256), 0, s, (const bf16_t*)x, ldx, N, HW, C, w, g_nchw, (bf16_t*)dx, lddx, part, (const bf16_t*)nullptr, 0, (const float*)nullptr, (const float*)nullptr, (const float*)nullptr, (const float*)nullptr, (float*)nullptr))
  } else {
    UZ_KOUT_SWITCH(Kout, hipLaunchKernelGGL((outconv_bwd_kernel<float, KOUT>), dim3((unsigned)g), dim3(256), 0, s, (const float*)x, ldx, N, HW, C, w, g_nchw, (float*)dx, lddx, part, (const float*)nullptr, 0, (const float*)nullptr, (const float*)nullptr, (const float*)nullptr, (const float*)nullptr, (float*)nullptr))
  }
  UZ_LAUNCH_CHECK("uz_outconv_bwd");
  const int ne = Kout * (C + 1);
  hipLaunchKernelGGL(outconv_bwd_finalize_kernel, dim3(uz_cdiv(ne, 32)), dim3(1024), 0, s, part, g, Kout, C, dw, db);
  UZ_LAUNCH_CHECK("uz_outconv_bwd(finalize)");
  return UZ_OK;
}

extern "C" int uz_colsum(int dtype, const void* x, int ld, int P, int C, float* out, void* stream) {
  UZ_REQUIRE(dtype == UZ_F32 || dtype == UZ_BF16, "uz_colsum: bad dtype");
  const int vec = dtype == UZ_BF16 ? 8 : 4;
  UZ_REQUIRE(x && out && P > 0 && C > 0 && C % vec == 0 && ld % vec == 0 && ld >= C, "uz_colsum: bad args");
  dim3 grid, block;
  reduce_shape(C / vec, P, &grid, &block);
  const size_t shm = (size_t)256 * vec * sizeof(float);
  hipStream_t s = (hipStream_t)stream;
  if (dtype == UZ_BF16)
    hipLaunchKernelGGL((colsum_kernel<bf16_t, false>), grid, block, shm, s, (const bf16_t*)x, ld, (long long)P, C, out);
  else
    hipLaunchKernelGGL((colsum_kernel<float, false>), grid, block, shm, s, (const float*)x, ld, (long long)P, C, out);
  UZ_LAUNCH_CHECK("uz_colsum");
  return UZ_OK;
}

extern "C" long long uz_colsum_workspace_bytes(int dtype, int P, int C) {
  UZ_REQUIRE(dtype == UZ_F32 || dtype == UZ_BF16, "uz_colsum_workspace_bytes: bad dtype");
  const int vec = dtype == UZ_BF16 ? 8 : 4;
  UZ_REQUIRE(P > 0 && C > 0 && C % vec == 0, "uz_colsum_workspace_bytes: bad shape");
  dim3 grid, block;
  reduce_shape(C / vec, P, &grid, &block);
  return (long long)grid.x * C * (long long)sizeof(float);
}

extern "C" int uz_colsum_ws(int dtype, const void* x, int ld, int P, int C, float* out, void* workspace,
                            void* stream) {
  UZ_REQUIRE(dtype == UZ_F32 || dtype == UZ_BF16, "uz_colsum_ws: bad dtype");
  const int vec = dtype == UZ_BF16 ? 8 : 4;
  UZ_REQUIRE(x && out && workspace && P > 0 && C > 0 && C % vec == 0 && ld % vec == 0 && ld >= C, "uz_colsum_ws: bad args");
  dim3 grid, block;
  reduce_shape(C / vec, P, &grid, &block);
  const size_t shm = (size_t)256 * vec * sizeof(float);
  hipStream_t s = (hipStream_t)stream;
  float* part = static_cast<float*>(workspace);
  if (dtype == UZ_BF16)
    hipLaunchKernelGGL((colsum_kernel<bf16_t, true>), grid, block, shm, s, (const bf16_t*)x, ld, (long long)P, C, part);
// ... 327 lines not shown
```

unet_zoo_amd/engine.py:

```python
from __future__ import annotations

import math
from typing import Callable, Dict, List, Optional, Sequence, Tuple

import torch
import torch.nn as nn

from . import _lib as L
from . import ops
from .ops import Act


def _round_up(a: int, b: int) -> int:
    return (a + b - 1) // b * b


class PackCache:

    def __init__(self):
        self.entries: Dict[tuple, tuple] = {}
        self._table: Optional[torch.Tensor] = None
        self._total = 0
        self._n = 0
        self._table_dtype = None
# ... 11 lines not shown
    def get(self, p: nn.Parameter, mode: int, kpad: int, dtype: torch.dtype) -> torch.Tensor:
        key = (id(p), mode, kpad, dtype)
        e = self.entries.get(key)
        if e is None:
            if mode == L.PACK_VEC_REPEAT:
                dst = p.detach().float().repeat(kpad).contiguous()
            else:
                dst = ops.pack_weights(p.detach(), mode, dtype, kpad)
            self.entries[key] = (p, mode, kpad, dtype, dst)
            self._table = None
            return dst
        return e[4]

    def refresh(self, dtype: torch.dtype) -> None:
        ents = [e for e in self.entries.values() if e[3] == dtype]
        if not ents:
            return
        if self._table is None or self._table_dtype != dtype:
            self._build_tables(ents, dtype)
        lib = L.load()
        if self._n3 > 0:
            L.check(lib.uz_pack_conv3x3_batched(L.dtype_code(dtype), self._table3.data_ptr(), self._n3,
                                                self._tiles3, L.stream_ptr()), "uz_pack_conv3x3_batched")
        if self._n > 0:
            L.check(lib.uz_pack_weights_batched(L.dtype_code(dtype), self._table.data_ptr(), self._n,
                                                self._total, L.stream_ptr()), "uz_pack_weights_batched")

    def _build_tables(self, ents, dtype) -> None:
        dev = ents[0][4].device
        tiled = {}
        generic = []
        for (p, mode, kpad, _, dst) in ents:
            ok = (mode in (L.PACK_CONV_FWD, L.PACK_CONV_DGRAD) and p.dim() == 4 and tuple(p.shape[2:]) == (3, 3)
                  and p.shape[0] % 32 == 0 and p.shape[1] % 32 == 0)
            if ok:
                it = tiled.setdefault(id(p), [p, None, None])
                it[1 if mode == L.PACK_CONV_FWD else 2] = dst
            else:
                generic.append((p, mode, kpad, dst))
        arr3 = (L.Pack3x3Item * max(len(tiled), 1))()
        tb = 0
        for i, (p, df, dd) in enumerate(tiled.values()):
            arr3[i] = L.Pack3x3Item(p.data_ptr(), df.data_ptr() if df is not None else None,
                                    dd.data_ptr() if dd is not None else None, p.shape[0], p.shape[1], tb, 0)
            tb += (p.shape[0] // 32) * (p.shape[1] // 32)
        self._n3, self._tiles3 = len(tiled), tb
        self._table3 = torch.frombuffer(bytearray(bytes(arr3)), dtype=torch.uint8).to(dev)
        arr = (L.PackItem * max(len(generic), 1))()
        begin = 0
        for i, (p, mode, kpad, dst) in enumerate(generic):
            if mode == L.PACK_VEC_REPEAT:
                arr[i] = L.PackItem(p.data_ptr(), dst.data_ptr(), begin, mode, p.numel(), 1, kpad, 0, 0)
                begin += dst.numel()
                continue
            d0, d1 = p.shape[0], p.shape[1]
            T = p.numel() // (d0 * d1)
            co, ci = (d0, d1) if mode in (L.PACK_CONV_FWD, L.PACK_CONV_DGRAD, L.PACK_IM2COL) else (d1, d0)
            arr[i] = L.PackItem(p.data_ptr(), dst.data_ptr(), begin, mode, co, ci, T, kpad, 0)
            begin += dst.numel()
        self._table = torch.frombuffer(bytearray(bytes(arr)), dtype=torch.uint8).to(dev)
        self._total, self._n, self._table_dtype = begin, len(generic), dtype

class ImageInput:

    __slots__ = ("nchw", "kpad", "dtype", "_patches", "N", "H", "W")

    def __init__(self, nchw: torch.Tensor, kpad: int, dtype: torch.dtype):
        self.nchw, self.kpad, self.dtype, self._patches = nchw, kpad, dtype, None
        self.N, _, self.H, self.W = nchw.shape

    def patches(self) -> Act:
        if self._patches is None:
            self._patches = ops.im2col3x3_nchw(self.nchw, self.kpad, self.dtype)
        return self._patches


class Engine:
    direct_first_conv = True
    defer_linear_wgrads = True
    fuse_bn_reduce = True
    fuse_bn_reduce_convt = True
    fold_bn_apply = True
    fold_bn_apply_head = True
    fuse_bn_finalize = False
    FIN_FLAGS = 4096
    reverse_element_passes = True

    def __init__(self, dtype: torch.dtype, device: torch.device, training: bool, record: bool,
                 grad_sink: Optional[Callable[[nn.Parameter, torch.Tensor], None]] = None,
                 pack_cache: Optional[PackCache] = None, grads_in_place: bool = False):
        self.dtype = dtype
        self.device = device
        self.training = training
        self.record = record
        self.tape: List[Callable[[], None]] = []
        self.param_grads: Dict[nn.Parameter, torch.Tensor] = {}
        self.grad_sink = grad_sink
        self.bk = 64 if dtype == torch.bfloat16 else 32
        self._bn_channels = 0
        self._sums: Optional[torch.Tensor] = None
        self._sums_used = 0
        self._cache = pack_cache if pack_cache is not None else PackCache()
        self.grads_in_place = grads_in_place
        self._heads: List[Tuple[Callable[..., None], int]] = []
        self.grad_log: List[Tuple[int, nn.Parameter]] = []
        self._pending_colsums: List[Tuple[int, nn.Parameter, Act]] = []
        self._pending_rowsums: List[Tuple[int, Callable[[], None]]] = []
        self._pending_wgrads: List[Tuple[int, nn.Parameter, Act, Act]] = []
        self._rowsum_items: list = []
        self._cpb: Dict[nn.Module, dict] = {}
        self._bn_counters: List[torch.Tensor] = []
        self._cur_entry = -1
        self._fin_flags: Optional[torch.Tensor] = None
        self._fin_used = 0

    def _fin_flag(self) -> Optional[torch.Tensor]:
        if not self.fuse_bn_finalize:
            return None
        if self._fin_flags is None:
            self._fin_flags = torch.zeros(self.FIN_FLAGS, dtype=torch.int32, device=self.device)
        if self._fin_used >= self.FIN_FLAGS:
            return None
        self._fin_used += 1
        return self._fin_flags[self._fin_used - 1:self._fin_used]

    def new_act(self, N, H, W, C, needs_grad=True) -> Act:
        return ops.new_act(N, H, W, C, self.dtype, self.device, needs_grad)

    def new_cat(self, N, H, W, channels: Sequence[int]) -> Tuple[Act, List[Act]]:
        full = self.new_act(N, H, W, sum(channels))
        parts, o = [], 0
        for c in channels:
            parts.append(full.window(o, c))
            o += c
        full.parts = parts
        return full, parts

    def _dst(self, p: nn.Parameter) -> Optional[torch.Tensor]:
        if self.grads_in_place and p.grad is not None and p.grad.is_contiguous() and p.grad.dtype == torch.float32:
            return p.grad
        return None

    def _give_grad(self, p: nn.Parameter, g: Optional[torch.Tensor]) -> None:
        if not isinstance(p, nn.Parameter):
            return
        self.grad_log.append((self._cur_entry, p))
        if self.grads_in_place and p.grad is not None:
            if g is None:
                return
            if p in self.param_grads:
                if g.data_ptr() == p.grad.data_ptr():
                    raise RuntimeError("a parameter shared by two layers received its second gradient in place: "
                                       "shared parameters are not supported by the in-place (graphed) backward")
                p.grad.add_(g.reshape(p.grad.shape))
            elif g.data_ptr() != p.grad.data_ptr():
                p.grad.copy_(g.reshape(p.grad.shape))
            self.param_grads[p] = None
            if self.grad_sink is not None:
                self.grad_sink(p, p.grad)
            return
        if g is None:
            g = torch.zeros(p.shape, dtype=torch.float32, device=self.device)
        if p in self.param_grads:
            self.param_grads[p] = self.param_grads[p] + g
        else:
            self.param_grads[p] = g
# ... 85 lines not shown
        Cout = conv.out_channels
        xf = getattr(x, "lazy", None)
        assert xf is None or (sole_reader and not im2col and conv.kernel_size == (3, 3) and conv.dilation == (1, 1)), \
            "a lazy activation goes to the 3x3 convolution it was deferred for"
        dil = conv.dilation[0]
        image = None
        if im2col and isinstance(x, ImageInput):
            if (self.direct_first_conv and conv.kernel_size == (3, 3) and dil == 1 and conv.padding == (1, 1)
                    and conv.stride == (1, 1) and ops.conv_first_supported(self.dtype, x.nchw.shape[1], Cout)):
                image = x.nchw
                image_version = image._version
            else:
                x = x.patches()
        if image is not None:
            wp, ntaps = None, 1
        elif im2col:
            wp = self._pack(conv.weight, L.PACK_IM2COL, x.C)
            ntaps = 1
        else:
            assert conv.kernel_size in ((3, 3), (1, 1)) and conv.in_channels == x.C
            wp = self._pack(conv.weight, L.PACK_CONV_FWD)
            ntaps = 9 if conv.kernel_size == (3, 3) else 1
            assert ntaps == 9 or not upsample
        y = self.new_act(N, H, W, Cout)
        bias = conv.bias.detach() if conv.bias is not None else None
        if image is not None:
            stats = ops.conv_first_fwd(image, conv.weight.detach(), bias, y, self.training)
        else:
            stats = ops.conv_igemm(x, wp, bias, y, ntaps=ntaps, dil=dil, taps_mode=tmode,
                                   want_stats=self.training, xform=xf)
        lazy = False
        if (defer_apply is not None and self.fold_bn_apply and out is None and not pool and residual is None and relu
                and stat_repeat == 1 and self.dtype == torch.bfloat16 and defer_apply.kernel_size == (3, 3)
                and defer_apply.dilation == (1, 1) and defer_apply.stride == (1, 1) and defer_apply.in_channels == Cout):
            c2 = defer_apply.out_channels
            lazy = (ops.conv_xform_supported(y, c2, c2)
                    and ops.wgrad_xform_shapes_supported(N, H, W, c2, c2, Cout, y.ld, self.dtype))
        elif (defer_apply is not None and self.fold_bn_apply and self.fold_bn_apply_head and out is None and not pool
                and residual is None and relu and stat_repeat == 1 and defer_apply.kernel_size == (1, 1)
                and defer_apply.in_channels == Cout and (self.training or not self.record)):
            lazy = self.fuse_bn_reduce_convt and ops.outconv_xform_supported(y, defer_apply.out_channels)
        fin = self._fin_flag() if (self.training and not lazy and stat_repeat == 1) else None
        vec = None
        if self.training:
            mom = bn.momentum if bn.momentum is not None else 0.1
            if fin is None:
                vec = ops.bn_finalize(stats if stat_repeat == 1 else stats * float(stat_repeat), y.P * stat_repeat,
                                      bn.weight.detach(), bn.bias.detach(), bn.eps, mom, bn.running_mean, bn.running_var)
            if bn.num_batches_tracked is not None:
                self._bn_counters.append(bn.num_batches_tracked)
        else:
            vec = self._bn_vectors(bn, None, y.P)
        if lazy:
            act = ops.Act(y.buf, y.off, y.C, N, H, W, True)
            act.lazy = (vec[0], vec[1])
            pooled = None
        else:
            act = out if out is not None else self.new_act(N, H, W, Cout)
            if pool and pool_ceil:
                pooled = self.new_act(N, (H + 1) // 2, (W + 1) // 2, Cout)
            else:
                pooled = self.new_act(N, H // 2, W // 2, Cout) if pool else None
            assert relu or residual is None
            if fin is not None:
                vec = ops.bn_relu_apply_fin(y, stats, y.P, bn.weight.detach(), bn.bias.detach(), bn.eps, mom, bn.running_mean,
                                            bn.running_var, fin, act, pooled, residual, pool_ceil, relu=relu)
            else:
                ops.bn_relu_apply(y, vec[0], vec[1], act, pooled, residual, pool_ceil, relu=relu,
                                  reverse=self.reverse_element_passes)
        if self.record and self.training and relu and pooled is None and residual is None and stat_repeat == 1:
            act.bn_src = (y, vec)

        frozen = not self.training
        if self.record:
            self._bn_channels += Cout

            def bwd():
                gs = self._sum_grads(act, 2)
                gp = self._sum_grads(pooled, 1)[0] if (pooled is not None and pooled.grads) else None
                g0 = gs[0] if len(gs) > 0 else None
                g1 = gs[1] if len(gs) > 1 else None
                if g0 is None and gp is None:
                    return
                if residual is not None:
                    if gp is not None or g1 is not None:
                        tot = self.new_act(N, H, W, Cout)
                        ops.pool_grad_combine(act, g0, g1, gp, tot, pool_ceil)
                        g0, g1, gp = tot, None, None
                    if residual.needs_grad:
                        residual.add_grad(g0)
                dy = self.new_act(N, H, W, Cout)
                dgamma, dbeta = self._dst(bn.weight), self._dst(bn.bias)
                if dgamma is None:
                    dgamma = torch.empty(Cout, dtype=torch.float32, device=self.device)
                if dbeta is None:
                    dbeta = torch.empty(Cout, dtype=torch.float32, device=self.device)
                parts = getattr(g0, "bn_partials", None) if (g1 is None and gp is None and residual is None) else None
                ops.bn_relu_bwd(y, vec, g0, g1, gp, self._bn_sums(Cout), dy, dgamma, dbeta, pool_ceil, relu=relu,
                                partials=parts, frozen=frozen, fin_flag=None if frozen else self._fin_flag(),
                                reverse=self.reverse_element_passes)
                self._give_grad(bn.weight, dgamma)
                self._give_grad(bn.bias, dbeta)
                if conv.bias is not None:
                    if frozen:
                        self._bias_grad(conv.bias, dy)
                    else:
                        self._give_grad(conv.bias, None)
                if image is not None:
                    if image._version != image_version:
                        raise RuntimeError("the network input was modified in place between forward and backward: the first "
                                           "convolution's weight gradient reads it (pass a copy, or finish backward first)")
                    self._give_grad(conv.weight, ops.conv_first_wgrad(image, dy, out=self._dst(conv.weight)))
                elif im2col:
                    dwp = ops.wgrad(dy, x, (Cout, x.C), ntaps=1)
                    cin = conv.in_channels
                    dw = dwp[:, :9 * cin].reshape(Cout, 9, cin).permute(0, 2, 1).reshape(conv.weight.shape)
                    self._give_grad(conv.weight, dw.contiguous())
                else:
                    if ntaps == 1 and tmode == L.TAPS_CONV:
                        self._linear_wgrad(conv.weight, dy, x)
                    else:
                        self._give_grad(conv.weight, ops.wgrad(dy, x, tuple(conv.weight.shape), ntaps=ntaps,
                                                               dil=dil, taps_mode=tmode,
                                                               out=self._dst(conv.weight), xform=xf))
                    if x.needs_grad and upsample:
                        du = self.new_act(N, H, W, x.C)
                        ops.conv_igemm(dy, self._pack(conv.weight, L.PACK_CONV_DGRAD), None, du,
                                       ntaps=9, dil=dil)
                        dx = self.new_act(x.N, x.H, x.W, x.C)
                        ops.sum2x2(du, dx)
                        x.add_grad(dx)
                    elif x.needs_grad:
                        dx = self.new_act(N, H, W, x.C)
                        want = x.parts is not None
                        src = getattr(x, "bn_src", None) if (sole_reader and not want and self.fuse_bn_reduce) else None
                        part = ops.conv_igemm(dy, self._pack(conv.weight, L.PACK_CONV_DGRAD), None, dx,
                                              ntaps=ntaps, dil=dil, want_stats=want, bnred=src)
                        if want:
                            dx.colsums = (part, 0)
                        elif src is not None and part is not None:
                            dx.bn_partials = part
                        x.add_grad(dx)

            self.tape.append(bwd)
        return act, pooled

    def attention_gate(self, g: Act, x: Act, blk: nn.Module, out: Act) -> Act:
        conv_g, bn_g = blk.w_g[0], blk.w_g[1]
        conv_x, bn_x = blk.w_x[0], blk.w_x[1]
        conv_q, bn_q = blk.psi[0], blk.psi[1]
        N, H, W, P = x.N, x.H, x.W, x.P
        Fi = conv_g.out_channels
        assert (g.N, g.H, g.W) == (N, H, W) and conv_q.out_channels == 1

        def conv1x1_bn(src: Act, conv: nn.Conv2d, bn: nn.BatchNorm2d):
            raw = self.new_act(N, H, W, conv.out_channels)
            st = ops.conv_igemm(src, self._pack(conv.weight, L.PACK_CONV_FWD),
                                conv.bias.detach() if conv.bias is not None else None, raw, ntaps=1,
                                want_stats=self.training)
            return raw, self._bn_vectors(bn, st, P)

        g1, vec_g = conv1x1_bn(g, conv_g, bn_g)
        x1, vec_x = conv1x1_bn(x, conv_x, bn_x)
        wpsi = conv_q.weight.detach().reshape(Fi)
        q, part = ops.attn_psi_fwd(g1, x1, vec_g, vec_x, wpsi,
                                   conv_q.bias.detach() if conv_q.bias is not None else None)
        vec_q = self._bn_vectors(bn_q, part, P)
        ops.attn_gate_fwd(x, q, vec_q, out)

        if self.record:
            frozen = not self.training

            def bwd():
                dout = self._sum_grads(out, 1)
                if not dout:
                    return
                dxd = self.new_act(N, H, W, x.C)
                dz, a01 = ops.attn_bwd_psi(dout[0], x, q, vec_q, dxd)
                dg1 = self.new_act(N, H, W, Fi)
                dx1 = self.new_act(N, H, W, Fi)
                tot = ops.attn_bwd_branches(g1, x1, q, dz, wpsi, vec_g, vec_x, vec_q, a01, dg1, dx1, frozen=frozen)
                totf, a01f = tot.float(), a01.float()
                self._give_grad(bn_q.weight, a01f[1:2])
                self._give_grad(bn_q.bias, a01f[0:1])
                self._give_grad(bn_g.weight, totf[Fi:2 * Fi])
                self._give_grad(bn_g.bias, totf[0:Fi])
                self._give_grad(bn_x.weight, totf[2 * Fi:3 * Fi])
                self._give_grad(bn_x.bias, totf[0:Fi].clone())
                self._give_grad(conv_q.weight, totf[3 * Fi:4 * Fi].reshape(conv_q.weight.shape))
                if frozen:
                    if conv_q.bias is not None:
                        self._give_grad(conv_q.bias, totf[4 * Fi:4 * Fi + 1].reshape(conv_q.bias.shape))
                    if conv_g.bias is not None:
                        self._bias_grad(conv_g.bias, dg1)
                    if conv_x.bias is not None:
# ... 1147 lines not shown
            self.tape.append(bwd)
        return dst

    def u2net_heads(self, feats: Sequence[Act], sides: Sequence[nn.Conv2d], fuse: nn.Conv2d) -> List[torch.Tensor]:
        N, H, W = feats[0].N, feats[0].H, feats[0].W
        S, K, HW = len(feats), sides[0].out_channels, H * W
        assert fuse.kernel_size == (1, 1) and fuse.in_channels == S * K and fuse.out_channels == K
        dev = self.device
        dcat = torch.empty((N, S * K, H, W), dtype=torch.float32, device=dev)
        taps = torch.empty(N * 9 * HW, dtype=torch.float32, device=dev)
        for s_, (f, conv) in enumerate(zip(feats, sides)):
            assert conv.kernel_size == (3, 3) and conv.padding == (1, 1) and conv.in_channels == f.C
            wt = conv.weight.detach()
            hw = f.H * f.W
            low = None if (f.H, f.W) == (H, W) else torch.empty((N, K, f.H, f.W), dtype=torch.float32, device=dev)
            for o in range(K):
                wp = wt.data_ptr() + o * f.C * 9 * 4
                bp = conv.bias.detach().data_ptr() + 4 * o if conv.bias is not None else None
                plane = dcat.data_ptr() + (s_ * K + o) * HW * 4
                if low is None:
                    ops.sideconv_fwd(f, wp, bp, taps, plane, S * K * HW)
                else:
                    lp = low.data_ptr() + o * hw * 4
                    ops.sideconv_fwd(f, wp, bp, taps, lp, K * hw)
                    ops.bilinear_planes(lp, K * hw, f.H, f.W, plane, S * K * HW, H, W, N)
        wf = fuse.weight.detach().reshape(K, S * K)
        d0 = ops.fuse1x1_fwd(dcat, wf, fuse.bias.detach() if fuse.bias is not None else None)
        outs = [d0] + [dcat[:, s_ * K:(s_ + 1) * K] for s_ in range(S)]

        if self.record:
            def bwd(*gs: Optional[torch.Tensor]):
                if all(g is None for g in gs):
                    return
                g0 = gs[0].contiguous().float() if gs[0] is not None else None
                extras = [g.contiguous().float() if g is not None else None for g in gs[1:]]
                dwf, dbf = self._dst(fuse.weight), (self._dst(fuse.bias) if fuse.bias is not None else None)
                if dwf is None:
                    dwf = torch.empty(fuse.weight.shape, dtype=torch.float32, device=dev)
                if dbf is None and fuse.bias is not None:
                    dbf = torch.empty(K, dtype=torch.float32, device=dev)
                dcat_g = ops.fuse1x1_bwd(dcat, wf, g0, extras, dwf, dbf)
                self._give_grad(fuse.weight, dwf)
                if fuse.bias is not None:
                    self._give_grad(fuse.bias, dbf)
                for s_, (f, conv) in enumerate(zip(feats, sides)):
                    hw = f.H * f.W
                    dw, db = self._dst(conv.weight), (self._dst(conv.bias) if conv.bias is not None else None)
                    if dw is None:
                        dw = torch.empty(conv.weight.shape, dtype=torch.float32, device=dev)
                    if db is None and conv.bias is not None:
                        db = torch.empty(K, dtype=torch.float32, device=dev)
                    low = None if (f.H, f.W) == (H, W) else torch.empty((N, K, f.H, f.W), dtype=torch.float32, device=dev)
                    wt = conv.weight.detach()
                    for o in range(K):
                        plane = dcat_g.data_ptr() + (s_ * K + o) * HW * 4
                        if low is None:
                            gp_, gi = plane, S * K * HW
                        else:
                            gp_, gi = low.data_ptr() + o * hw * 4, K * hw
                            ops.bilinear_planes(plane, S * K * HW, f.H, f.W, gp_, gi, H, W, N, backward=True)
                        dx = self.new_act(f.N, f.H, f.W, f.C) if f.needs_grad else None
                        ops.sideconv_bwd(f, wt.data_ptr() + o * f.C * 9 * 4, gp_, gi, dx,
                                         dw.data_ptr() + o * f.C * 9 * 4,
                                         db.data_ptr() + 4 * o if db is not None else None)
                        if dx is not None:
                            f.add_grad(dx)
                    self._give_grad(conv.weight, dw)
                    if conv.bias is not None:
                        self._give_grad(conv.bias, db)

            self._heads.append((bwd, len(outs)))
        return outs

    def out_conv(self, x: Act, conv: nn.Conv2d, sole_reader: bool = False) -> torch.Tensor:
        assert conv.kernel_size == (1, 1) and conv.in_channels == x.C
        K = conv.out_channels
        w = conv.weight.detach().reshape(K, x.C)
        b = conv.bias.detach() if conv.bias is not None else torch.zeros(K, device=self.device)
        xf = getattr(x, "lazy", None)
        assert xf is None or sole_reader, "a lazy activation goes to the head it was deferred for"
        logits = ops.outconv_fwd(x, w, b, xform=xf)
        if self.record:
            def bwd(g_logits: torch.Tensor):
                dx = self.new_act(x.N, x.H, x.W, x.C) if (x.needs_grad or xf is not None) else None
                dwt = self._dst(conv.weight)
                dbt = self._dst(conv.bias) if conv.bias is not None else None
                src = getattr(x, "bn_src", None) if (sole_reader and (self.fuse_bn_reduce_convt or xf is not None)) else None
                dw, db = ops.outconv_bwd(x, w, g_logits.contiguous().float(), dx,
                                         dwt.view(K, x.C) if dwt is not None else None, dbt, bnred=src, lazy=xf is not None)
                self._give_grad(conv.weight, dwt if dwt is not None else dw.reshape(conv.weight.shape))
                if conv.bias is not None:
                    self._give_grad(conv.bias, db)
                if dx is not None:
                    x.add_grad(dx)

            self._heads.append((bwd, 1))
        return logits

    def out_conv_resized(self, x: Act, conv: nn.Conv2d, H: int, W: int, align_corners: bool = True) -> torch.Tensor:
        low = self.out_conv(x, conv)
        N, K, h, w = low.shape
        logits = torch.empty((N, K, H, W), dtype=torch.float32, device=low.device)
        ops.bilinear_planes_ac(low.data_ptr(), h, w, logits.data_ptr(), H, W, N * K, align_corners)
        if self.record:
            inner, n = self._heads.pop()

            def bwd(g_logits: torch.Tensor):
                g_low = torch.empty((N, K, h, w), dtype=torch.float32, device=low.device)
                ops.bilinear_planes_ac(g_logits.contiguous().float().data_ptr(), h, w, g_low.data_ptr(), H, W, N * K,
                                       align_corners, backward=True)
                inner(g_low)

            self._heads.append((bwd, n))
        return logits

    def layer_norm_head(self, x: Act, ln: nn.LayerNorm, conv: nn.Conv2d, *, mode: int = L.LN_PLAIN, r: int = 1) -> torch.Tensor:
        C, K = ln.normalized_shape[0], conv.out_channels
        assert conv.kernel_size == (1, 1) and conv.in_channels == C
        if not ops.ln_head_supported(C, K, self.dtype):
            return self.out_conv(self.layer_norm(x, ln, mode=mode, r=r), conv)
        if mode == L.LN_EXPAND:
            assert x.C == r * r * C
            N, Ho, Wo = x.N, x.H * r, x.W * r
        else:
            assert mode == L.LN_PLAIN and x.C == C
            N, Ho, Wo = x.N, x.H, x.W
        gamma, beta = ln.weight.detach(), ln.bias.detach()
        w = conv.weight.detach().reshape(K, C)
        b = conv.bias.detach() if conv.bias is not None else None
        logits, stats = ops.ln_head_fwd(x, gamma, beta, w, b, N, Ho, Wo, C, mode=mode, r=r, eps=ln.eps)
        if self.record:
            def bwd(g_logits: torch.Tensor):
                dx = self.new_act(x.N, x.H, x.W, x.C)
                dwt = self._dst(conv.weight)
                outs = ops.ln_head_bwd(x, gamma, beta, w, stats, g_logits.contiguous().float(), dx, mode=mode, r=r,
                                       eps=ln.eps, dgamma=self._dst(ln.weight), dbeta=self._dst(ln.bias),
                                       dw=dwt.view(K, C) if dwt is not None else None,
                                       db=self._dst(conv.bias) if conv.bias is not None else None)
                self._give_grad(conv.weight, dwt if dwt is not None else outs[2].reshape(conv.weight.shape))
                if conv.bias is not None:
                    self._give_grad(conv.bias, outs[3])
                self._give_grad(ln.weight, outs[0])
                self._give_grad(ln.bias, outs[1])
                if x.needs_grad:
                    x.add_grad(dx)

            self._heads.append((bwd, 1))
        return logits

    def conv5x5(self, x: Act, conv: nn.Conv2d) -> Tuple[Act, torch.Tensor]:
        assert conv.kernel_size == (5, 5) and conv.padding == (2, 2) and conv.stride == (1, 1) and conv.dilation == (1, 1) \
            and conv.groups == 1 and conv.in_channels == x.C
        N, H, W, Cout = x.N, x.H, x.W, conv.out_channels
        thin = Cout % 8 != 0
        if thin:
            y = Act(torch.zeros((x.P, _round_up(Cout, 8)), dtype=self.dtype, device=self.device), 0, Cout, N, H, W)
        else:
            y = self.new_act(N, H, W, Cout)
        stats = ops.conv5x5(x, self._pack(conv.weight, L.PACK_CONV_FWD), conv.bias.detach() if conv.bias is not None else None,
                            y, want_stats=True)
        if self.record:
            def bwd():
                g = self._total_grad(y)
                if g is None:
                    return
                if conv.bias is not None:
                    self._give_grad(conv.bias, None)
                if thin:
                    assert g.off == 0 and g.ld == _round_up(Cout, 8)
                    g = Act(g.buf, 0, g.ld, N, H, W)
                self._give_grad(conv.weight, ops.wgrad5x5(g, x, tuple(conv.weight.shape), out=self._dst(conv.weight)))
                if x.needs_grad:
                    if thin:
                        wd = torch.zeros((x.C, 25, g.C), dtype=torch.float32, device=self.device)
                        wd[:, :, :Cout] = conv.weight.detach().flip(2, 3).reshape(Cout, x.C, 25).permute(1, 2, 0)
                        wd = wd.reshape(x.C, 25 * g.C).to(self.dtype)
# ... 89 lines not shown
```

unet_zoo_amd/ops.py:

```python
from __future__ import annotations

from ctypes import byref
from typing import List, Optional, Sequence

import math

import torch

from . import _lib as L


class Act:

    __slots__ = ("buf", "off", "C", "N", "H", "W", "grads", "parts", "rparts", "needs_grad", "colsums", "bn_src",
                 "bn_partials", "lazy")

    def __init__(self, buf: torch.Tensor, off: int, C: int, N: int, H: int, W: int,
                 needs_grad: bool = True):
        assert buf.dim() == 2 and buf.is_contiguous() and buf.shape[0] == N * H * W
        assert 0 <= off and off + C <= buf.shape[1]
        self.buf, self.off, self.C, self.N, self.H, self.W = buf, off, C, N, H, W
        self.grads: List["Act"] = []
        self.parts: Optional[Sequence["Act"]] = None
        self.rparts: Optional[Sequence[tuple]] = None
# ... 141 lines not shown
    def __exit__(self, *exc):
        if _prof_on:
            n = L.load().uz_profile_disarm()
            if n == 0:
                self.e1.record()
            _prof_log.append((self.name, self.e0, self.e1, self.flops, self.bytes, _prof_scope))
        return False


def _tname(dt: torch.dtype) -> str:
    return "bf16" if dt == torch.bfloat16 else "f32"


def pack_weights(w: torch.Tensor, mode: int, dtype: torch.dtype, kpad: int = 0) -> torch.Tensor:
    L.require_cuda(w)
    assert w.dtype == torch.float32 and w.is_contiguous()
    d0, d1 = w.shape[0], w.shape[1]
    T = w.numel() // (d0 * d1)
    if mode in (L.PACK_CONV_FWD, L.PACK_CONV_DGRAD, L.PACK_IM2COL):
        Co, Ci = d0, d1
    else:
        Ci, Co = d0, d1
    if mode == L.PACK_CONV_FWD:
        shape = (Co, T * Ci)
    elif mode == L.PACK_CONV_DGRAD:
        shape = (Ci, T * Co)
    elif mode == L.PACK_CONVT_FWD:
        shape = (T * Co, Ci)
    elif mode == L.PACK_CONVT_DGRAD:
        shape = (Ci, T * Co)
    else:
        shape = (Co, kpad)
    dst = torch.empty(shape, dtype=dtype, device=w.device)
    L.check(L.load().uz_pack_weights(L.dtype_code(dtype), mode, w.data_ptr(), Co, Ci, T, kpad,
                                     dst.data_ptr(), L.stream_ptr()), "uz_pack_weights")
    return dst


def im2col3x3_nchw(x: torch.Tensor, kpad: int, dtype: torch.dtype) -> Act:
    L.require_cuda(x)
    assert x.dtype == torch.float32 and x.is_contiguous() and x.dim() == 4
    N, C, H, W = x.shape
    out = new_act(N, H, W, kpad, dtype, x.device, needs_grad=False)
    with _Timed("im2col3x3_nchw", 0.0, 4.0 * x.numel() + out.buf.element_size() * out.buf.numel()):
        L.check(L.load().uz_im2col3x3_nchw(L.dtype_code(dtype), x.data_ptr(), N, C, H, W, kpad,
                                           out.buf.data_ptr(), L.stream_ptr()), "uz_im2col3x3_nchw")
    return out


def conv_first_supported(dtype: torch.dtype, C: int, Cout: int) -> bool:
    return bool(L.load().uz_conv3x3_first_supported(L.dtype_code(dtype), C, Cout))


def conv_first_fwd(x: torch.Tensor, w: torch.Tensor, bias: Optional[torch.Tensor], y: Act, want_stats: bool):
    L.require_cuda(x, w, y.buf)
    assert x.dtype == torch.float32 and x.is_contiguous() and w.dtype == torch.float32 and w.is_contiguous()
    N, C, H, W = x.shape
    Cout = w.shape[0]
    assert (y.N, y.H, y.W, y.C) == (N, H, W, Cout) and tuple(w.shape) == (Cout, C, 3, 3)
    lib = L.load()
    stats = None
    if want_stats:
        rows = L.check_count(lib.uz_conv3x3_first_rows(N, H, W), "uz_conv3x3_first_rows")
        stats = torch.empty((rows, 2, Cout), dtype=torch.float32, device=x.device)
    with _Timed("conv3x3_first_bf16", 2.0 * N * H * W * 9 * C * Cout, 4.0 * x.numel() + 2.0 * y.P * Cout):
        L.check(lib.uz_conv3x3_first_fwd(L.dtype_code(y.dtype), x.data_ptr(), N, C, H, W, w.data_ptr(), _p(bias), Cout,
                                         y.ptr(), y.ld, _p(stats), L.stream_ptr()), "uz_conv3x3_first_fwd")
    return stats


def conv_first_wgrad(x: torch.Tensor, dy: Act, out: Optional[torch.Tensor] = None) -> torch.Tensor:
    L.require_cuda(x, dy.buf)
    N, C, H, W = x.shape
    Cout = dy.C
    lib = L.load()
    ws_bytes = L.check_count(lib.uz_conv3x3_first_wgrad_workspace_bytes(N, H, W, Cout), "uz_conv3x3_first_wgrad_workspace_bytes")
    ws = torch.empty(ws_bytes // 4, dtype=torch.float32, device=x.device)
    if out is None:
        out = torch.empty((Cout, C, 3, 3), dtype=torch.float32, device=x.device)
    assert out.numel() == Cout * C * 9 and out.is_contiguous() and out.dtype == torch.float32
    with _Timed("wgrad_first_bf16", 2.0 * N * H * W * 9 * C * Cout, 4.0 * x.numel() + 2.0 * dy.P * Cout):
        L.check(lib.uz_conv3x3_first_wgrad(L.dtype_code(dy.dtype), x.data_ptr(), N, C, H, W, dy.ptr(), dy.ld, Cout,
                                           out.data_ptr(), ws.data_ptr(), L.stream_ptr()), "uz_conv3x3_first_wgrad")
    return out


def conv_kernel_name(d, with_workspace: bool = False) -> str:
    import ctypes
    buf = ctypes.create_string_buffer(96)
    L.check_count(L.load().uz_conv_igemm_kernel_name(byref(d), 1 if with_workspace else 0, buf, 96),
                  "uz_conv_igemm_kernel_name")
    return buf.value.decode()


def conv_igemm(x: Act, w_packed: torch.Tensor, bias: Optional[torch.Tensor], y: Act, *,
               ntaps: int, dil: int = 1, taps_mode: int = L.TAPS_CONV,
               store_mode: int = L.STORE_PLAIN, nout: Optional[int] = None, co: int = 0,
               want_stats: bool = False, res: Optional[Act] = None,
               bnred: Optional[tuple] = None, xform: Optional[tuple] = None) -> Optional[torch.Tensor]:
    L.require_cuda(x.buf, w_packed, y.buf)
    lib = L.load()
    if taps_mode == L.TAPS_CONV:
        N, H, W = x.N, x.H, x.W
    elif taps_mode == L.TAPS_CONV_UP2:
        N, H, W = x.N, 2 * x.H, 2 * x.W
    elif taps_mode == L.TAPS_CONV_S2:
        N, H, W = x.N, (x.H + 1) // 2, (x.W + 1) // 2
    else:
        N, H, W = x.N, x.H // 2, x.W // 2
    shuffle = store_mode == L.STORE_SHUFFLE2X2
    d = L.ConvDesc(L.dtype_code(x.dtype), N, H, W, x.H, x.W, x.C, x.ld,
                   nout if nout is not None else y.C, y.ld, ntaps, taps_mode, dil, store_mode, co,
                   y.H if shuffle else 0, y.W if shuffle else 0)
    assert w_packed.dtype == x.dtype and y.dtype == x.dtype
    assert w_packed.shape == (d.Nout, ntaps * x.C), (tuple(w_packed.shape), d.Nout, ntaps, x.C)
    stats = None
    if want_stats:
        gm = L.check_count(lib.uz_conv_igemm_ws_grid_m(byref(d)), "uz_conv_igemm_ws_grid_m")
        stats = torch.empty((gm, 2, d.Nout), dtype=torch.float32, device=x.buf.device)
    wsb = L.check_count(lib.uz_conv_igemm_workspace_bytes(byref(d)), "uz_conv_igemm_workspace_bytes")
    ws = torch.empty(wsb // 4, dtype=torch.float32, device=x.buf.device) if wsb > 0 else None
    M, K, es = N * H * W, ntaps * x.C, x.buf.element_size()
    kname = conv_kernel_name(d, ws is not None)
    if xform is not None:
        assert bnred is None and res is None
        with _Timed(kname + "_xf", 2.0 * M * d.Nout * K, es * (x.P * x.C + M * d.Nout + d.Nout * K)):
            L.check(lib.uz_conv_igemm_xf(byref(d), x.ptr(), xform[0].data_ptr(), xform[1].data_ptr(), w_packed.data_ptr(),
                                         _p(bias), y.ptr(), _p(stats), L.stream_ptr()), "uz_conv_igemm_xf")
        return stats
    if bnred is not None:
        assert bias is None and res is None and not want_stats
        bn_y, vec4 = bnred
        if not lib.uz_conv_igemm_bnred_supported(byref(d)) or (bn_y.P, bn_y.C) != (y.P, y.C):
            bnred = None
        else:
            gm = L.check_count(lib.uz_conv_igemm_grid_m(byref(d)), "uz_conv_igemm_grid_m")
            part = torch.empty((gm, 2, d.Nout), dtype=torch.float32, device=x.buf.device)
            with _Timed(kname + "_bnred", 2.0 * M * d.Nout * K, es * (x.P * x.C + 2 * M * d.Nout + d.Nout * K)):
                L.check(lib.uz_conv_igemm_bnred(byref(d), x.ptr(), w_packed.data_ptr(), y.ptr(), bn_y.ptr(), bn_y.ld,
                                                vec4[0].data_ptr(), vec4[1].data_ptr(), vec4[2].data_ptr(),
                                                vec4[3].data_ptr(), part.data_ptr(), L.stream_ptr()),
                        "uz_conv_igemm_bnred")
            return part
    if res is not None:
        assert (res.P, res.C) == (y.P, y.C) and res.dtype == y.dtype and not want_stats
        if kname.startswith("gemm_dma") and store_mode == L.STORE_PLAIN:
            with _Timed(kname, 2.0 * M * d.Nout * K, es * (x.P * x.C + 2 * M * d.Nout + d.Nout * K)):
                L.check(lib.uz_conv_igemm_res_ws(byref(d), x.ptr(), w_packed.data_ptr(), _p(bias), res.ptr(), res.ld, y.ptr(),
                                                 _p(ws), L.stream_ptr()), "uz_conv_igemm_res_ws")
            return None
    with _Timed(kname, 2.0 * M * d.Nout * K,
                        es * (x.P * x.C + M * d.Nout + d.Nout * K)):
        L.check(lib.uz_conv_igemm_ws(byref(d), x.ptr(), w_packed.data_ptr(), _p(bias), y.ptr(), _p(stats),
                                     _p(ws), L.stream_ptr()), "uz_conv_igemm_ws")
    if res is not None:
        add_acts(y, res, y)
    return stats


def conv_xform_supported(x: Act, nout: int, ldy: int, *, upsample: bool = False) -> bool:
    H, W = (2 * x.H, 2 * x.W) if upsample else (x.H, x.W)
    d = L.ConvDesc(L.dtype_code(x.dtype), x.N, H, W, x.H, x.W, x.C, x.ld, nout, ldy, 9,
                   L.TAPS_CONV_UP2 if upsample else L.TAPS_CONV, 1, L.STORE_PLAIN, 0, 0, 0)
    return bool(L.load().uz_conv_igemm_xf_supported(byref(d)))


# ... 86 lines not shown


def colstats(x: Act) -> torch.Tensor:
    lib = L.load()
    code = L.dtype_code(x.dtype)
    rows = L.check_count(lib.uz_colstats_rows(code, x.P, x.C), "uz_colstats_rows")
    part = torch.empty((rows, 2, x.C), dtype=torch.float32, device=x.buf.device)
    with _Timed("colstats", 0.0, x.buf.element_size() * x.P * x.C):
        L.check(lib.uz_colstats(code, x.ptr(), x.ld, x.P, x.C, part.data_ptr(), L.stream_ptr()), "uz_colstats")
    return part


def add_acts(a: Act, b: Act, out: Act) -> None:
    pool_grad_combine(a, a, b, None, out)


def add_relu(a: Act, b: Optional[Act], out: Act) -> None:
    assert (a.P, a.C) == (out.P, out.C) and (b is None or (b.P, b.C) == (a.P, a.C))
    with _Timed("add_relu", 0.0, a.buf.element_size() * a.P * a.C * (2 + (b is not None))):
        L.check(L.load().uz_add_relu(L.dtype_code(a.dtype), a.ptr(), a.ld, b.ptr() if b is not None else None,
                                     b.ld if b is not None else 0, out.ptr(), out.ld, a.P, a.C, L.stream_ptr()), "uz_add_relu")


def relu_bwd(out: Act, g: Act, dx: Act) -> None:
    assert (out.P, out.C) == (g.P, g.C) == (dx.P, dx.C)
    with _Timed("relu_bwd", 0.0, out.buf.element_size() * out.P * out.C * 3):
        L.check(L.load().uz_relu_bwd(L.dtype_code(out.dtype), out.ptr(), out.ld, g.ptr(), g.ld, dx.ptr(), dx.ld, out.P,
                                     out.C, L.stream_ptr()), "uz_relu_bwd")


def bn_eval_scale(gamma, beta, running_mean, running_var, eps: float):
    lib = L.load()
    C = gamma.numel()
    vec = torch.empty((2, C), dtype=torch.float32, device=gamma.device)
    L.check(lib.uz_bn_eval_scale(C, gamma.data_ptr(), beta.data_ptr(), running_mean.data_ptr(),
                                 running_var.data_ptr(), eps, vec[0].data_ptr(), vec[1].data_ptr(),
                                 L.stream_ptr()), "uz_bn_eval_scale")
    return vec


def bn_relu_apply(y: Act, scale: torch.Tensor, shift: torch.Tensor, act: Act,
                  pooled: Optional[Act] = None, res: Optional[Act] = None, pool_ceil: bool = False,
                  relu: bool = True, reverse: bool = False) -> None:
    if pooled is not None:
        want = ((y.H + 1) // 2, (y.W + 1) // 2) if pool_ceil else (y.H // 2, y.W // 2)
        assert (pooled.H, pooled.W) == want, (pooled.H, pooled.W, want)
    lib = L.load()
    es = y.buf.element_size()
    with _Timed("bn_relu_apply", 0.0, es * y.P * y.C * ((2.25 if pooled is not None else 2.0) + (res is not None))):
        L.check(lib.uz_bn_relu_add_apply(L.dtype_code(y.dtype), y.ptr(), y.ld, scale.data_ptr(),
                                         shift.data_ptr(), y.N, y.H, y.W, y.C,
                                         res.ptr() if res is not None else None,
                                         res.ld if res is not None else 0, act.ptr(), act.ld,
                                         pooled.ptr() if pooled is not None else None,
                                         pooled.ld if pooled is not None else 0,
                                         int(pool_ceil) | (0 if relu else 2) | (4 if reverse else 0), L.stream_ptr()),
                "uz_bn_relu_add_apply")


def bn_relu_apply_fin(y: Act, stats: torch.Tensor, count: int, gamma, beta, eps: float, momentum: float, running_mean,
                      running_var, flag: torch.Tensor, act: Act, pooled: Optional[Act] = None, res: Optional[Act] = None,
                      pool_ceil: bool = False, relu: bool = True) -> torch.Tensor:
    if pooled is not None:
        want = ((y.H + 1) // 2, (y.W + 1) // 2) if pool_ceil else (y.H // 2, y.W // 2)
        assert (pooled.H, pooled.W) == want, (pooled.H, pooled.W, want)
    C = stats.shape[2]
    assert C == y.C and flag.dtype == torch.int32 and flag.numel() == 1
    vec = torch.empty((4, C), dtype=torch.float32, device=stats.device)
    es = y.buf.element_size()
    with _Timed("bn_relu_apply", 0.0, es * y.P * y.C * ((2.25 if pooled is not None else 2.0) + (res is not None)) + 4.0 * stats.numel()):
        L.check(L.load().uz_bn_relu_add_apply_fin(
            L.dtype_code(y.dtype), y.ptr(), y.ld, stats.data_ptr(), stats.shape[0], float(count), gamma.data_ptr(), beta.data_ptr(),
            eps, momentum, _p(running_mean), _p(running_var), vec.data_ptr(), flag.data_ptr(), y.N, y.H, y.W, y.C,
            res.ptr() if res is not None else None, res.ld if res is not None else 0, act.ptr(), act.ld,
            pooled.ptr() if pooled is not None else None, pooled.ld if pooled is not None else 0,
            int(pool_ceil) | (0 if relu else 2), L.stream_ptr()), "uz_bn_relu_add_apply_fin")
    return vec


BN_BWD_ALTERNATE = True


def bn_relu_bwd(y: Act, vec: torch.Tensor, g0: Optional[Act], g1: Optional[Act],
                gpool: Optional[Act], sums: torch.Tensor, dy: Act, dgamma: torch.Tensor,
                dbeta: torch.Tensor, pool_ceil: bool = False, relu: bool = True,
                partials: Optional[torch.Tensor] = None, frozen: bool = False,
                fin_flag: Optional[torch.Tensor] = None, reverse: bool = False) -> None:
    lib = L.load()
    def desc(rev):
        return L.BnBwdDesc(L.dtype_code(y.dtype), y.N, y.H, y.W, y.C, y.ld,
                           g0.ld if g0 is not None else 0, g1.ld if g1 is not None else 0,
                           gpool.ld if gpool is not None else 0, dy.ld,
                           int(pool_ceil) | (0 if relu else 2) | (4 if rev else 0))
    d = desc(reverse)
    d_apply = desc(reverse != (partials is None and BN_BWD_ALTERNATE))
    args = (y.ptr(), vec[0].data_ptr(), vec[1].data_ptr(), vec[2].data_ptr(), vec[3].data_ptr(),
            g0.ptr() if g0 is not None else None, g1.ptr() if g1 is not None else None,
            gpool.ptr() if gpool is not None else None)
    s = L.stream_ptr()
    nsrc = (g0 is not None) + (g1 is not None) + 0.25 * (gpool is not None)
    es = y.buf.element_size()
    if fin_flag is not None and not frozen:
        if partials is not None:
            assert relu and g1 is None and gpool is None and partials.shape[1:] == (2, y.C) and partials.is_contiguous()
            rows, pptr = partials.shape[0], partials.data_ptr()
        else:
            wsb = L.check_count(lib.uz_bn_relu_bwd_workspace_bytes(byref(d), int(gpool is not None)),
                                "uz_bn_relu_bwd_workspace_bytes")
            ws = torch.empty(wsb // 4, dtype=torch.float32, device=y.buf.device)
            rows, pptr = wsb // (8 * y.C), ws.data_ptr()
            with _Timed("bn_relu_bwd_reduce", 0.0, es * y.P * y.C * (1 + nsrc)):
                L.check(lib.uz_bn_relu_bwd_reduce_rows(byref(d), *args, pptr, s), "uz_bn_relu_bwd_reduce_rows")
        with _Timed("bn_relu_bwd_apply", 0.0, es * y.P * y.C * (2 + nsrc)):
            L.check(lib.uz_bn_relu_bwd_apply_fin(byref(d_apply), *args, pptr, rows, sums.data_ptr(), dgamma.data_ptr(),
                                                 dbeta.data_ptr(), fin_flag.data_ptr(), float(y.P), dy.ptr(), s),
                    "uz_bn_relu_bwd_apply_fin")
        return
    if partials is not None:
        assert relu and g1 is None and gpool is None and partials.shape[1:] == (2, y.C) and partials.is_contiguous()
        L.check(lib.uz_bn_bwd_finalize(partials.data_ptr(), partials.shape[0], y.C, sums.data_ptr(),
                                       dgamma.data_ptr(), dbeta.data_ptr(), s), "uz_bn_bwd_finalize")
    else:
        wsb = L.check_count(lib.uz_bn_relu_bwd_workspace_bytes(byref(d), int(gpool is not None)),
                            "uz_bn_relu_bwd_workspace_bytes")
        ws = torch.empty(wsb // 4, dtype=torch.float32, device=y.buf.device)
        with _Timed("bn_relu_bwd_reduce", 0.0, es * y.P * y.C * (1 + nsrc)):
            L.check(lib.uz_bn_relu_bwd_reduce(byref(d), *args, ws.data_ptr(), sums.data_ptr(),
                                              dgamma.data_ptr(), dbeta.data_ptr(), s), "uz_bn_relu_bwd_reduce")
    if frozen:
        sums.zero_()
    with _Timed("bn_relu_bwd_apply", 0.0, es * y.P * y.C * (2 + nsrc)):
        L.check(lib.uz_bn_relu_bwd_apply(byref(d_apply), *args, sums.data_ptr(), float(y.P), dy.ptr(), s),
                "uz_bn_relu_bwd_apply")


def outconv_xform_supported(x: Act, K: int) -> bool:
    return x.dtype == torch.bfloat16 and x.C % 8 == 0 and x.C // 8 <= 64 and 1 <= K <= 8 and x.ld % 8 == 0


def outconv_fwd(x: Act, w: torch.Tensor, b: torch.Tensor, xform: Optional[tuple] = None) -> torch.Tensor:
    lib = L.load()
    K = w.shape[0]
    out = torch.empty((x.N, K, x.H, x.W), dtype=torch.float32, device=x.buf.device)
    if xform is not None:
        assert outconv_xform_supported(x, K)
        L.check(lib.uz_outconv_fwd_xf(L.dtype_code(x.dtype), x.ptr(), x.ld, x.N, x.H * x.W, x.C, xform[0].data_ptr(),
                                      xform[1].data_ptr(), w.data_ptr(), b.data_ptr(), K, out.data_ptr(), L.stream_ptr()),
                "uz_outconv_fwd_xf")
        return out
    L.check(lib.uz_outconv_fwd(L.dtype_code(x.dtype), x.ptr(), x.ld, x.N, x.H * x.W, x.C,
                               w.data_ptr(), b.data_ptr(), K, out.data_ptr(), L.stream_ptr()),
            "uz_outconv_fwd")
    return out


def outconv_bwd(x: Act, w: torch.Tensor, g: torch.Tensor, dx: Optional[Act],
                dw: Optional[torch.Tensor] = None, db: Optional[torch.Tensor] = None,
                bnred: Optional[tuple] = None, lazy: bool = False):
    lib = L.load()
    K = w.shape[0]
    assert g.dtype == torch.float32 and g.is_contiguous() and g.shape == (x.N, K, x.H, x.W)
    dev = x.buf.device
    if dw is None:
        dw = torch.empty((K, x.C), dtype=torch.float32, device=dev)
    if db is None:
        db = torch.empty(K, dtype=torch.float32, device=dev)
    code = L.dtype_code(x.dtype)
    wsb = L.check_count(lib.uz_outconv_bwd_workspace_bytes(code, x.N, x.H * x.W, x.C, K),
                        "uz_outconv_bwd_workspace_bytes")
    ws = torch.empty(wsb // 4, dtype=torch.float32, device=dev)
    if lazy:
        assert bnred is not None and dx is not None and x.dtype == torch.bfloat16 and (bnred[0].P, bnred[0].C) == (x.P, x.C), \
            "a head on a lazy activation takes its backward through uz_outconv_bwd_bnred"
    if bnred is not None and dx is not None and x.dtype == torch.bfloat16 and (bnred[0].P, bnred[0].C) == (x.P, x.C):
        bn_y, vec4 = bnred
        rows = L.check_count(lib.uz_outconv_bwd_rows(code, x.N, x.H * x.W, x.C), "uz_outconv_bwd_rows")
        part = torch.empty((rows, 2, x.C), dtype=torch.float32, device=dev)
        L.check(lib.uz_outconv_bwd_bnred(code, None if lazy else x.ptr(), x.ld, x.N, x.H * x.W, x.C, w.data_ptr(), K, g.data_ptr(),
                                         dx.ptr(), dx.ld, dw.data_ptr(), db.data_ptr(), ws.data_ptr(), bn_y.ptr(), bn_y.ld,
                                         vec4[0].data_ptr(), vec4[1].data_ptr(), vec4[2].data_ptr(), vec4[3].data_ptr(),
                                         part.data_ptr(), L.stream_ptr()), "uz_outconv_bwd_bnred")
        dx.bn_partials = part
        return dw.view(K, x.C), db
    L.check(lib.uz_outconv_bwd(code, x.ptr(), x.ld, x.N, x.H * x.W, x.C, w.data_ptr(), K, g.data_ptr(),
                               dx.ptr() if dx is not None else None,
                               dx.ld if dx is not None else 0, dw.data_ptr(), db.data_ptr(),
                               ws.data_ptr(), L.stream_ptr()), "uz_outconv_bwd")
    return dw.view(K, x.C), db


def colsum(x: Act, out: Optional[torch.Tensor] = None) -> torch.Tensor:
    lib = L.load()
    code = L.dtype_code(x.dtype)
    if out is None:
        out = torch.empty(x.C, dtype=torch.float32, device=x.buf.device)
    assert out.numel() == x.C and out.dtype == torch.float32 and out.is_contiguous()
    wsb = L.check_count(lib.uz_colsum_workspace_bytes(code, x.P, x.C), "uz_colsum_workspace_bytes")
    ws = torch.empty(wsb // 4, dtype=torch.float32, device=x.buf.device)
    with _Timed("colsum", 0.0, x.buf.element_size() * x.P * x.C):
        L.check(lib.uz_colsum_ws(code, x.ptr(), x.ld, x.P, x.C, out.data_ptr(), ws.data_ptr(), L.stream_ptr()),
                "uz_colsum_ws")
    return out


def colsum_batched(pairs: Sequence) -> None:
    by_dtype = {}
    for x, out in pairs:
        assert out.numel() == x.C and out.dtype == torch.float32 and out.is_contiguous()
        by_dtype.setdefault(x.dtype, []).append((x, out))
    lib = L.load()
    for dt, group in by_dtype.items():
        arr = (L.ColsumItem * len(group))()
        nbytes = 0.0
        for i, (x, out) in enumerate(group):
            arr[i] = L.ColsumItem(x.ptr(), out.data_ptr(), x.P, x.C, x.ld, 0)
            nbytes += x.buf.element_size() * x.P * x.C
        code = L.dtype_code(dt)
        wsb = L.check_count(lib.uz_colsum_batched_workspace_bytes(code, arr, len(group)), "uz_colsum_batched_workspace_bytes")
        ws = torch.empty(max(wsb // 4, 1), dtype=torch.float32, device=group[0][0].buf.device)
        with _Timed("colsum_batched", 0.0, nbytes):
            L.check(lib.uz_colsum_batched(code, arr, len(group), ws.data_ptr(), L.stream_ptr()), "uz_colsum_batched")


def sum_rows(partial: torch.Tensor, rows: int, n: int) -> torch.Tensor:
    out = torch.empty(n, dtype=torch.float64, device=partial.device)
    L.check(L.load().uz_sum_rows(partial.data_ptr(), rows, n, out.data_ptr(), L.stream_ptr()), "uz_sum_rows")
    return out


def sum_rows_f32_batched(entries: Sequence) -> None:
    if not entries:
        return
    arr = (L.SumRowsItem * len(entries))()
    for i, (partial, rows, out0, out1) in enumerate(entries):
        n0 = out0.numel()
        n = n0 + (out1.numel() if out1 is not None else 0)
        assert partial.numel() == rows * n and partial.dtype == torch.float32
        arr[i] = L.SumRowsItem(partial.data_ptr(), out0.data_ptr(), out1.data_ptr() if out1 is not None else None, rows, n, n0, 0)
    with _Timed("sum_rows_batched", 0.0, 4.0 * sum(e[0].numel() for e in entries)):
        L.check(L.load().uz_sum_rows_f32_batched(arr, len(entries), L.stream_ptr()), "uz_sum_rows_f32_batched")


def sum_rows_f32(partial: torch.Tensor, rows: int, out0: torch.Tensor, out1: Optional[torch.Tensor] = None,
                 defer: Optional[list] = None) -> None:
    if defer is not None:
        defer.append((partial, rows, out0, out1))
        return
    n0 = out0.numel()
    n = n0 + (out1.numel() if out1 is not None else 0)
    assert partial.numel() == rows * n and partial.dtype == torch.float32
    for o in (out0, out1):
        assert o is None or (o.dtype == torch.float32 and o.is_contiguous())
    L.check(L.load().uz_sum_rows_f32(partial.data_ptr(), rows, n, out0.data_ptr(), n0,
                                     out1.data_ptr() if out1 is not None else None, L.stream_ptr()), "uz_sum_rows_f32")


def attn_grid(dtype: torch.dtype, P: int, channels: int) -> int:
    return L.check_count(L.load().uz_attn_grid(L.dtype_code(dtype), P, channels), "uz_attn_grid")


def attn_psi_fwd(g1: Act, x1: Act, vec_g, vec_x, wpsi: torch.Tensor, bpsi: Optional[torch.Tensor]):
    dev = g1.buf.device
    G = attn_grid(g1.dtype, g1.P, g1.C)
    q = torch.empty(g1.P, dtype=torch.float32, device=dev)
# ... 661 lines not shown
```

Before: 2511 images/sec.

## Fuse BN-ReLU backward into head gradient and first-conv weight-gradient kernels

The head output conv's backward can now skip storing its input-gradient activation. Instead it hands a virtual HeadGrad (upstream gradient, weights, BN partials) down the graph, and a new kernel recomputes g·w inline while applying the BN-ReLU backward. The first 3x3 conv's weight-gradient kernel gains a BN variant that reads the raw activation and the upstream gradient and applies the BN-ReLU backward transform while staging dy into LDS. This removes one full write and read of an intermediate gradient tensor. The cost is more register pressure (waves_per_eu pinned to 3) and extra activation loads inside the wgrad kernel.

```diff
diff --git a/include/unetzoo_hip.h b/include/unetzoo_hip.h
--- a/include/unetzoo_hip.h
+++ b/include/unetzoo_hip.h
@@ -111,6 +111,9 @@
 long long uz_conv3x3_first_wgrad_workspace_bytes(int N, int H, int W, int Cout);
 int uz_conv3x3_first_wgrad(int dtype, const float* x, int N, int C, int H, int W, const void* dy, int lddy, int Cout, float* dw,
                            void* workspace, void* stream);
+int uz_conv3x3_first_wgrad_bn(int dtype, const float* x, int N, int C, int H, int W, const void* g, int ldg, const void* y,
+                              int ldy, const float* scale, const float* shift, const float* mean, const float* invstd,
+                              const double* sums, double count, int Cout, float* dw, void* workspace, void* stream);
 
 enum { UZ_PACK_CONV_FWD = 0, UZ_PACK_CONV_DGRAD = 1, UZ_PACK_CONVT_FWD = 2, UZ_PACK_CONVT_DGRAD = 3,
        UZ_PACK_IM2COL = 4, UZ_PACK_VEC_REPEAT = 5 };
@@ -182,6 +185,10 @@
                              const float* partial, int rows, double* sums, float* dgamma, float* dbeta, int* flag,
                              double count, void* dy, void* stream);
 int uz_bn_bwd_finalize(const float* partial, int rows, int C, double* sums, float* dgamma, float* dbeta, void* stream);
+int uz_bn_relu_bwd_apply_head_supported(int dtype, int C, int Kout);
+int uz_bn_relu_bwd_apply_head(const uz_bnbwd_desc* d, const void* y, const float* scale, const float* shift, const float* mean,
+                              const float* invstd, const float* g_nchw, const float* w, int Kout, const double* sums,
+                              double count, void* dy, void* stream);
 
 int uz_outconv_fwd(int dtype, const void* x, int ldx, int N, int HW, int C, const float* w,
                    const float* b, int Kout, float* out_nchw, void* stream);
diff --git a/unet_zoo_amd/_lib.py b/unet_zoo_amd/_lib.py
--- a/unet_zoo_amd/_lib.py
+++ b/unet_zoo_amd/_lib.py
@@ -17,9 +17,9 @@
 EXPORTS = (
     "uz_abi_version", "uz_last_error_string", "uz_build_ablate", "uz_source_hash", "uz_set_cu_reserve", "uz_get_cu_reserve", "uz_clock_probe", "uz_conv_igemm_grid_m", "uz_conv_igemm",
     "uz_wgrad_split", "uz_wgrad_workspace_bytes", "uz_wgrad", "uz_wgrad_kernel_name", "uz_wgrad_phase", "uz_wgrad_xf_supported", "uz_wgrad_xf", "uz_conv3x3_first_supported", "uz_conv3x3_first_rows", "uz_conv3x3_first_fwd",
-    "uz_conv3x3_first_wgrad_workspace_bytes", "uz_conv3x3_first_wgrad", "uz_pack_weights", "uz_pack_weights_batched", "uz_pack_conv3x3_batched", "uz_im2col3x3_nchw", "uz_bn_finalize",
+    "uz_conv3x3_first_wgrad_workspace_bytes", "uz_conv3x3_first_wgrad", "uz_conv3x3_first_wgrad_bn", "uz_pack_weights", "uz_pack_weights_batched", "uz_pack_conv3x3_batched", "uz_im2col3x3_nchw", "uz_bn_finalize",
     "uz_bn_eval_scale", "uz_bn_relu_apply", "uz_bn_relu_bwd_workspace_bytes", "uz_bn_relu_bwd_reduce", "uz_bn_relu_bwd_apply",
-    "uz_outconv_fwd", "uz_outconv_fwd_xf", "uz_outconv_bwd_workspace_bytes", "uz_outconv_bwd", "uz_outconv_bwd_rows", "uz_outconv_bwd_bnred",
+    "uz_outconv_fwd", "uz_outconv_fwd_xf", "uz_outconv_bwd_workspace_bytes", "uz_outconv_bwd", "uz_outconv_bwd_rows", "uz_outconv_bwd_bnred", "uz_bn_relu_bwd_apply_head_supported", "uz_bn_relu_bwd_apply_head",
     "uz_colsum",
     "uz_attn_grid", "uz_attn_psi_fwd", "uz_attn_gate_fwd", "uz_attn_bwd_psi", "uz_attn_bwd_reduce",
     "uz_attn_bwd_apply", "uz_sum_rows", "uz_sum_rows_f32", "uz_sum2x2",
@@ -202,6 +202,7 @@
     lib.uz_conv3x3_first_wgrad_workspace_bytes.argtypes = [ip, ip, ip, ip]
     lib.uz_conv3x3_first_wgrad_workspace_bytes.restype = ctypes.c_longlong
     lib.uz_conv3x3_first_wgrad.argtypes = [ip, vp, ip, ip, ip, ip, vp, ip, ip, vp, vp, vp]
+    lib.uz_conv3x3_first_wgrad_bn.argtypes = [ip, vp, ip, ip, ip, ip, vp, ip, vp, ip, vp, vp, vp, vp, vp, ctypes.c_double, ip, vp, vp, vp]
     lib.uz_pack_weights.argtypes = [ip, ip, vp, ip, ip, ip, ip, vp, vp]
     lib.uz_pack_weights_batched.argtypes = [ip, vp, ip, ctypes.c_longlong, vp]
     lib.uz_pack_conv3x3_batched.argtypes = [ip, vp, ip, ip, vp]
@@ -219,6 +220,8 @@
     lib.uz_outconv_bwd_workspace_bytes.argtypes = [ip, ip, ip, ip, ip]
     lib.uz_outconv_bwd.argtypes = [ip, vp, ip, ip, ip, ip, vp, ip, vp, vp, ip, vp, vp, vp, vp]
     lib.uz_outconv_bwd_rows.argtypes = [ip, ip, ip, ip]
+    lib.uz_bn_relu_bwd_apply_head_supported.argtypes = [ip, ip, ip]
+    lib.uz_bn_relu_bwd_apply_head.argtypes = [POINTER(BnBwdDesc), vp, vp, vp, vp, vp, vp, vp, ip, vp, ctypes.c_double, vp, vp]
     lib.uz_outconv_bwd_bnred.argtypes = [ip, vp, ip, ip, ip, ip, vp, ip, vp, vp, ip, vp, vp, vp, vp, ip, vp, vp, vp, vp, vp, vp]
     lib.uz_colsum.argtypes = [ip, vp, ip, ip, ip, vp, vp]
     lib.uz_colsum_workspace_bytes.argtypes = [ip, ip, ip]
diff --git a/unet_zoo_amd/csrc/uz_conv_first.hip b/unet_zoo_amd/csrc/uz_conv_first.hip
--- a/unet_zoo_amd/csrc/uz_conv_first.hip
+++ b/unet_zoo_amd/csrc/uz_conv_first.hip
@@ -14,6 +14,14 @@
   const void* dy;
   float* slab;
   int N, C, H, W, Cout, ldy, th_n, tw_n, ntiles;
+  const void* yraw;
+  const float* bn_scale;
+  const float* bn_shift;
+  const float* bn_mean;
+  const float* bn_invstd;
+  const double* bn_sums;
+  double inv_count;
+  int ldyr;
 };
 
 __device__ __forceinline__ float round_bf16(float v) { return (float)(bf16_t)v; }
@@ -181,10 +189,11 @@
   }
 }
 
-template <int CT>
-__global__ __launch_bounds__(256) void conv_first_wgrad_kernel(const CfArgs a) {
+template <int CT, bool BN>
+__device__ __forceinline__ void conv_first_wgrad_body(const CfArgs& a) {
   constexpr int RB = CT * 64;
   __shared__ float sx[3 * PH * PW];
+  __shared__ __attribute__((aligned(16))) float sbn[BN ? 6 : 1][64];
   __shared__ __attribute__((aligned(16))) char sdy[TH * TW * RB];
   static_assert(4 * CT * 16 * 64 * 4 == TH * TW * RB, "the waves' accumulators meet in the dy tile's LDS");
   float (*sacc)[CT][16][64] = reinterpret_cast<float (*)[CT][16][64]>(sdy);
@@ -193,6 +202,18 @@
   const int per = a.th_n * a.tw_n;
   const int K = a.C * 9;
   const bf16_t* dyg = static_cast<const bf16_t*>(a.dy);
+  const bf16_t* yrg = static_cast<const bf16_t*>(a.yraw);
+  if constexpr (BN) {
+    if (tid < 64) {
+      const int c = tid < a.Cout ? tid : 0;
+      sbn[0][tid] = a.bn_scale[c];
+      sbn[1][tid] = a.bn_shift[c];
+      sbn[2][tid] = a.bn_mean[c];
+      sbn[3][tid] = a.bn_invstd[c];
+      sbn[4][tid] = (float)(a.bn_sums[c] * a.inv_count);
+      sbn[5][tid] = (float)(a.bn_sums[a.Cout + c] * a.inv_count);
+    }
+  }
 
   const int k = l31;
   const int kc = k / 9, kt = k - kc * 9, kty = kt / 3, ktx = kt - kty * 3;
@@ -210,7 +231,7 @@
   constexpr int CPP = RB / 16;
   constexpr int NDY = TH * TW * CPP / 256;
   float hreg[4];
-  f32x4 dreg[NDY];
+  f32x4 dreg[NDY], yreg[BN ? NDY : 1];
   unsigned hmask = 0, dmask = 0;
   auto dy_fetch = [&](int tile) __attribute__((always_inline)) {
     const int img = tile / per, rem = tile - img * per;
@@ -222,6 +243,7 @@
       const int r = p / TW, c = p % TW, gh = h0 + r, gw = w0 + c;
       const bool ok = gh < a.H && gw < a.W && ch * 8 < a.Cout;
       dreg[j] = *reinterpret_cast<const f32x4*>(ok ? dyg + (((size_t)img * a.H + gh) * a.W + gw) * a.ldy + ch * 8 : dyg);
+      if constexpr (BN) yreg[j] = *reinterpret_cast<const f32x4*>(ok ? yrg + (((size_t)img * a.H + gh) * a.W + gw) * a.ldyr + ch * 8 : yrg);
       dmask |= ok ? 1u << j : 0u;
     }
   };
@@ -233,14 +255,45 @@
   for (int tile = blockIdx.x; tile < a.ntiles; tile += gridDim.x) {
     __syncthreads();
     halo_store(sx, hreg, hmask, tid, a.C * PH * PW);
-#pragma unroll
-    for (int j = 0; j < NDY; ++j) {
-      const int idx = tid + 256 * j;
-      const int p = idx / CPP, ch = idx % CPP;
-      const int gran = ch >> 2, sw = (p >> 1) & 1;
-      const int pg = (CT == 2) ? (gran ^ sw) : gran;
-      const f32x4 z4 = {0.f, 0.f, 0.f, 0.f};
-      *reinterpret_cast<f32x4*>(sdy + p * RB + pg * 64 + (ch & 3) * 16) = (dmask >> j & 1u) ? dreg[j] : z4;
+    if constexpr (!BN) {
+#pragma unroll
+      for (int j = 0; j < NDY; ++j) {
+        const int idx = tid + 256 * j;
+        const int p = idx / CPP, ch = idx % CPP;
+        const int gran = ch >> 2, sw = (p >> 1) & 1;
+        const int pg = (CT == 2) ? (gran ^ sw) : gran;
+        const f32x4 z4 = {0.f, 0.f, 0.f, 0.f};
+        *reinterpret_cast<f32x4*>(sdy + p * RB + pg * 64 + (ch & 3) * 16) = (dmask >> j & 1u) ? dreg[j] : z4;
+      }
+    } else {
+      typedef __attribute__((ext_vector_type(2))) float f32x2;
+#pragma unroll
+      for (int hf = 0; hf < 2; ++hf) {
+        const int c4 = (tid % CPP) * 8 + 4 * hf;
+        const f32x4 bsc = *reinterpret_cast<const f32x4*>(&sbn[0][c4]), bsh = *reinterpret_cast<const f32x4*>(&sbn[1][c4]);
+        const f32x4 bmu = *reinterpret_cast<const f32x4*>(&sbn[2][c4]), bis = *reinterpret_cast<const f32x4*>(&sbn[3][c4]);
+        const f32x4 bk0 = *reinterpret_cast<const f32x4*>(&sbn[4][c4]), bk1 = *reinterpret_cast<const f32x4*>(&sbn[5][c4]);
+#pragma unroll
+        for (int j = 0; j < NDY; ++j) {
+          const int idx = tid + 256 * j;
+          const int p = idx / CPP, ch = idx % CPP;
+          const int gran = ch >> 2, sw = (p >> 1) & 1;
+          const int pg = (CT == 2) ? (gran ^ sw) : gran;
+          const f32x2 graw = {dreg[j][2 * hf], dreg[j][2 * hf + 1]}, yraw = {yreg[j][2 * hf], yreg[j][2 * hf + 1]};
+          const bf16x4 gv4 = __builtin_bit_cast(bf16x4, graw), yv4 = __builtin_bit_cast(bf16x4, yraw);
+          bf16x4 o4;
+#pragma unroll
+          for (int i = 0; i < 4; ++i) {
+            const float yv = (float)yv4[i], gv = (float)gv4[i];
+            const float pre = fmaf(yv, bsc[i], bsh[i]);
+            const float dz = pre > 0.f ? gv : 0.f;
+            const float xh = (yv - bmu[i]) * bis[i];
+            o4[i] = (bf16_t)(bsc[i] * (dz - bk0[i] - xh * bk1[i]));
+          }
+          const bf16x4 z4 = {(bf16_t)0.f, (bf16_t)0.f, (bf16_t)0.f, (bf16_t)0.f};
+          *reinterpret_cast<bf16x4*>(sdy + p * RB + pg * 64 + (ch & 3) * 16 + 8 * hf) = (dmask >> j & 1u) ? o4 : z4;
+        }
+      }
     }
     __syncthreads();
     {
@@ -282,6 +335,15 @@
     const int co = 32 * t + (r & 3) + 8 * (r >> 2) + 4 * (l >> 5), kk = l & 31;
     if (co < a.Cout) a.slab[((size_t)blockIdx.x * a.Cout + co) * 32 + kk] = s;
   }
+}
+
+template <int CT>
+__global__ __launch_bounds__(256) void conv_first_wgrad_kernel(const CfArgs a) {
+  conv_first_wgrad_body<CT, false>(a);
+}
+template <int CT>
+__global__ __launch_bounds__(256) __attribute__((amdgpu_waves_per_eu(3, 3))) void conv_first_wgrad_bn_kernel(const CfArgs a) {
+  conv_first_wgrad_body<CT, true>(a);
 }
 
 __global__ __launch_bounds__(256) void conv_first_wgrad_reduce_kernel(const float* __restrict__ slab, int nwg, int Cout, int K,
@@ -376,6 +438,39 @@
   return (long long)first_wgrad_grid(ntiles) * Cout * 32 * (long long)sizeof(float);
 }
 
+extern "C" int uz_conv3x3_first_wgrad_bn(int dtype, const float* x, int N, int C, int H, int W, const void* g, int ldg,
+                                         const void* y, int ldy, const float* scale, const float* shift, const float* mean,
+                                         const float* invstd, const double* sums, double count, int Cout, float* dw,
+                                         void* workspace, void* stream) {
+  int rc = check(dtype, N, C, H, W, Cout, ldg, "uz_conv3x3_first_wgrad_bn");
+  if (rc == UZ_OK) rc = check(dtype, N, C, H, W, Cout, ldy, "uz_conv3x3_first_wgrad_bn");
+  if (rc != UZ_OK) return rc;
+  UZ_REQUIRE(x && g && y && dw && workspace && ((uintptr_t)g & 15) == 0 && ((uintptr_t)y & 15) == 0,
+             "uz_conv3x3_first_wgrad_bn: null / unaligned pointer");
+  UZ_REQUIRE(scale && shift && mean && invstd && sums && count > 0, "uz_conv3x3_first_wgrad_bn: BatchNorm vectors / count");
+  CfArgs a = {};
+  a.x = x;
+  a.dy = g;
+  a.yraw = y;
+  a.ldyr = ldy;
+  a.bn_scale = scale;
+  a.bn_shift = shift;
+  a.bn_mean = mean;
+  a.bn_invstd = invstd;
+  a.bn_sums = sums;
+  a.inv_count = 1.0 / count;
+  a.slab = static_cast<float*>(workspace);
+  fill(a, N, C, H, W, Cout, ldg);
+  const int grid = first_wgrad_grid(a.ntiles);
+  hipStream_t s = static_cast<hipStream_t>(stream);
+  if (Cout == 64) hipLaunchKernelGGL(conv_first_wgrad_bn_kernel<2>, dim3(grid), dim3(256), 0, s, a);
+  else hipLaunchKernelGGL(conv_first_wgrad_bn_kernel<1>, dim3(grid), dim3(256), 0, s, a);
+  UZ_LAUNCH_CHECK("uz_conv3x3_first_wgrad_bn");
+  hipLaunchKernelGGL(conv_first_wgrad_reduce_kernel, dim3(Cout * 32 / 16), dim3(256), 0, s, a.slab, grid, Cout, C * 9, dw);
+  UZ_LAUNCH_CHECK("uz_conv3x3_first_wgrad_bn(reduce)");
+  return UZ_OK;
+}
+
 extern "C" int uz_conv3x3_first_wgrad(int dtype, const float* x, int N, int C, int H, int W, const void* dy, int lddy,
                                       int Cout, float* dw, void* workspace, void* stream) {
   const int rc = check(dtype, N, C, H, W, Cout, lddy, "uz_conv3x3_first_wgrad");
diff --git a/unet_zoo_amd/csrc/uz_eltwise.hip b/unet_zoo_amd/csrc/uz_eltwise.hip
--- a/unet_zoo_amd/csrc/uz_eltwise.hip
+++ b/unet_zoo_amd/csrc/uz_eltwise.hip
@@ -520,6 +520,88 @@
         const int which = e / VEC, ch = c0 + (e % VEC);
         a.partials[((size_t)blockIdx.x * 2 + which) * a.C + ch] = t;
       }
+    }
+  }
+}
+
+struct BnBwdHeadArgs {
+  const bf16_t* y;
+  bf16_t* dy;
+  const float* scale;
+  const float* shift;
+  const float* mean;
+  const float* invstd;
+  const double* sums;
+  const float* g;
+  const float* w;
+  double inv_count;
+  int P, HW, C, ldy, lddy, rev;
+};
+
+template <int KOUT>
+__global__ __launch_bounds__(256) void bn_relu_bwd_head_kernel(const BnBwdHeadArgs a) {
+  typedef bf16_t T;
+  constexpr int VEC = ElemTraits<T>::VEC, NPIX = 4;
+  const T* __restrict__ y = a.y;
+  const float* __restrict__ g = a.g;
+  T* __restrict__ dy = a.dy;
+  const int CC = a.C / VEC;
+  const int cc = blockIdx.y * blockDim.x + threadIdx.x;
+  const bool cok = cc < CC;
+  const int c0 = (cok ? cc : 0) * VEC;
+  const long long units = a.P;
+
+  float sc[VEC], sh[VEC], mu[VEC], is[VEC], k0[VEC], k1[VEC], wr[KOUT][VEC];
+#pragma unroll
+  for (int i = 0; i < VEC; ++i) {
+    sc[i] = a.scale[c0 + i];
+    sh[i] = a.shift[c0 + i];
+    mu[i] = a.mean[c0 + i];
+    is[i] = a.invstd[c0 + i];
+    k0[i] = (float)(a.sums[c0 + i] * a.inv_count);
+    k1[i] = (float)(a.sums[a.C + c0 + i] * a.inv_count);
+#pragma unroll
+    for (int k = 0; k < KOUT; ++k) wr[k][i] = a.w[k * a.C + c0 + i];
+  }
+  const long long ustride = (long long)gridDim.x * blockDim.y;
+  const bool rev = a.rev != 0;
+  for (long long u0 = (long long)blockIdx.x * blockDim.y + threadIdx.y; u0 < units && cok; u0 += NPIX * ustride) {
+    size_t pix[NPIX];
+    bool in[NPIX];
+#pragma unroll
+    for (int k = 0; k < NPIX; ++k) {
+      const long long q = u0 + k * ustride;
+      in[k] = q < units;
+      pix[k] = (size_t)(in[k] ? (rev ? units - 1 - q : q) : units - 1);
+    }
+    Vec16<T> yr[NPIX];
+    float gq[NPIX][KOUT];
+#pragma unroll
+    for (int k = 0; k < NPIX; ++k) {
+      yr[k] = ld16(y + pix[k] * a.ldy + c0);
+      const int p = (int)pix[k];
+      const int img = (KOUT == 1) ? 0 : p / a.HW;
+      const int hw = p - img * a.HW;
+#pragma unroll
+      for (int kk = 0; kk < KOUT; ++kk) gq[k][kk] = g[((size_t)img * KOUT + kk) * a.HW + hw];
+    }
+#pragma unroll
+    for (int k = 0; k < NPIX; ++k) {
+      if (!in[k]) continue;
+      float out[VEC];
+#pragma unroll
+      for (int i = 0; i < VEC; ++i) {
+        float d = 0.f;
+#pragma unroll
+        for (int kk = 0; kk < KOUT; ++kk) d = fmaf(gq[k][kk], wr[kk][i], d);
+        const float gv = (float)(T)d;
+        const float yv = (float)yr[k].v[i];
+        const float pre = fmaf(yv, sc[i], sh[i]);
+        const float dz = pre > 0.f ? gv : 0.f;
+        const float xh = (yv - mu[i]) * is[i];
+        out[i] = sc[i] * (dz - k0[i] - xh * k1[i]);
+      }
+      store_f(dy + pix[k] * a.lddy + c0, out);
     }
   }
 }
@@ -1501,6 +1583,46 @@
                              : bnbwd_launch<float, 2, true>(d, a, gpool != nullptr, s);
 }
 
+extern "C" int uz_bn_relu_bwd_apply_head_supported(int dtype, int C, int Kout) {
+  return dtype == UZ_BF16 && C > 0 && C % 8 == 0 && Kout >= 1 && Kout <= OUTCONV_MAXK;
+}
+
+extern "C" int uz_bn_relu_bwd_apply_head(const uz_bnbwd_desc* d, const void* y, const float* scale, const float* shift,
+                                         const float* mean, const float* invstd, const float* g_nchw, const float* w,
+                                         int Kout, const double* sums, double count, void* dy, void* stream) {
+  UZ_REQUIRE(d != nullptr, "uz_bn_relu_bwd_apply_head: null descriptor");
+  UZ_REQUIRE(uz_bn_relu_bwd_apply_head_supported(d->dtype, d->C, Kout), "uz_bn_relu_bwd_apply_head: dtype=%d C=%d Kout=%d unsupported",
+             d->dtype, d->C, Kout);
+  UZ_REQUIRE(y && scale && shift && mean && invstd && g_nchw && w && sums && dy, "uz_bn_relu_bwd_apply_head: null pointer");
+  UZ_REQUIRE(d->N > 0 && d->H > 0 && d->W > 0 && (long long)d->N * d->H * d->W < (1LL << 31), "uz_bn_relu_bwd_apply_head: bad shape");
+  UZ_REQUIRE(d->ldy % 8 == 0 && d->ldy >= d->C && d->lddy % 8 == 0 && d->lddy >= d->C, "uz_bn_relu_bwd_apply_head: bad ldy / lddy");
+  UZ_REQUIRE((d->pool_ceil & 3) == 0, "uz_bn_relu_bwd_apply_head: a ReLU block without a pool only");
+  UZ_REQUIRE(count > 0, "uz_bn_relu_bwd_apply_head: count");
+  BnBwdHeadArgs a;
+  a.y = static_cast<const bf16_t*>(y);
+  a.dy = static_cast<bf16_t*>(dy);
+  a.scale = scale;
+  a.shift = shift;
+  a.mean = mean;
+  a.invstd = invstd;
+  a.sums = sums;
+  a.g = g_nchw;
+  a.w = w;
+  a.inv_count = 1.0 / count;
+  a.P = d->N * d->H * d->W;
+  a.HW = d->H * d->W;
+  a.C = d->C;
+  a.ldy = d->ldy;
+  a.lddy = d->lddy;
+  a.rev = (d->pool_ceil & 4) != 0;
+  dim3 grid, block;
+  bnbwd_shape(d, false, &grid, &block, 2);
+  hipStream_t s = (hipStream_t)stream;
+  UZ_KOUT_SWITCH(Kout, hipLaunchKernelGGL((bn_relu_bwd_head_kernel<KOUT>), grid, block, 0, s, a))
+  UZ_LAUNCH_CHECK("uz_bn_relu_bwd_apply_head");
+  return UZ_OK;
+}
+
 extern "C" int uz_outconv_fwd(int dtype, const void* x, int ldx, int N, int HW, int C, const float* w,
                               const float* b, int Kout, float* out_nchw, void* stream) {
   UZ_REQUIRE(dtype == UZ_F32 || dtype == UZ_BF16, "uz_outconv_fwd: bad dtype");
@@ -1566,11 +1688,11 @@
                                     const float* shift, const float* mean, const float* invstd, float* bn_partial,
                                     void* stream) {
   UZ_REQUIRE(dtype == UZ_BF16, "uz_outconv_bwd_bnred: bf16 only");
-  UZ_REQUIRE(w && g_nchw && dw && db && workspace && dx && bn_y && scale && shift && mean && invstd && bn_partial,
+  UZ_REQUIRE(w && g_nchw && dw && db && workspace && bn_y && scale && shift && mean && invstd && bn_partial,
              "uz_outconv_bwd_bnred: null pointer");
   UZ_REQUIRE(Kout >= 1 && Kout <= OUTCONV_MAXK, "uz_outconv_bwd_bnred: Kout=%d", Kout);
   UZ_REQUIRE(C % 8 == 0 && C / 8 <= 64, "uz_outconv_bwd_bnred: C=%d unsupported", C);
-  UZ_REQUIRE((x == nullptr || (ldx % 8 == 0 && ldx >= C)) && lddx % 8 == 0 && lddx >= C && ld_bny % 8 == 0 && ld_bny >= C && N > 0 &&
+  UZ_REQUIRE((x == nullptr || (ldx % 8 == 0 && ldx >= C)) && (dx == nullptr || (lddx % 8 == 0 && lddx >= C)) && ld_bny % 8 == 0 && ld_bny >= C && N > 0 &&
                  HW > 0 && (long long)N * HW < (1LL << 31), "uz_outconv_bwd_bnred: bad shape");
   const int g = outconv_bwd_grid(dtype, N, HW, C);
   float* part = static_cast<float*>(workspace);
diff --git a/unet_zoo_amd/engine.py b/unet_zoo_amd/engine.py
--- a/unet_zoo_amd/engine.py
+++ b/unet_zoo_amd/engine.py
@@ -117,6 +117,8 @@
     fuse_bn_reduce_convt = True
     fold_bn_apply = True
     fold_bn_apply_head = True
+    fold_head_grad = True
+    fold_first_bn_bwd = True
     fuse_bn_finalize = False
     FIN_FLAGS = 4096
     reverse_element_passes = True
@@ -368,6 +370,8 @@
                 g1 = gs[1] if len(gs) > 1 else None
                 if g0 is None and gp is None:
                     return
+                head = isinstance(g0, ops.HeadGrad)
+                assert not head or (g1 is None and gp is None and residual is None and relu and not frozen and pooled is None)
                 if residual is not None:
                     if gp is not None or g1 is not None:
                         tot = self.new_act(N, H, W, Cout)
@@ -375,16 +379,23 @@
                         g0, g1, gp = tot, None, None
                     if residual.needs_grad:
                         residual.add_grad(g0)
-                dy = self.new_act(N, H, W, Cout)
+                fold_first = (self.fold_first_bn_bwd and image is not None and not frozen and relu and not head
+                              and self.dtype == torch.bfloat16 and pooled is None and residual is None and g1 is None
+                              and gp is None and not self.fuse_bn_finalize)
+                dy = None if fold_first else self.new_act(N, H, W, Cout)
                 dgamma, dbeta = self._dst(bn.weight), self._dst(bn.bias)
                 if dgamma is None:
                     dgamma = torch.empty(Cout, dtype=torch.float32, device=self.device)
                 if dbeta is None:
                     dbeta = torch.empty(Cout, dtype=torch.float32, device=self.device)
-                parts = getattr(g0, "bn_partials", None) if (g1 is None and gp is None and residual is None) else None
-                ops.bn_relu_bwd(y, vec, g0, g1, gp, self._bn_sums(Cout), dy, dgamma, dbeta, pool_ceil, relu=relu,
-                                partials=parts, frozen=frozen, fin_flag=None if frozen else self._fin_flag(),
-                                reverse=self.reverse_element_passes)
+                sums = self._bn_sums(Cout)
+                if head:
+                    ops.bn_relu_bwd_head(y, vec, g0, sums, dy, dgamma, dbeta, reverse=self.reverse_element_passes)
+                else:
+                    parts = getattr(g0, "bn_partials", None) if (g1 is None and gp is None and residual is None) else None
+                    ops.bn_relu_bwd(y, vec, g0, g1, gp, sums, dy, dgamma, dbeta, pool_ceil, relu=relu,
+                                    partials=parts, frozen=frozen, fin_flag=None if frozen else self._fin_flag(),
+                                    reverse=self.reverse_element_passes)
                 self._give_grad(bn.weight, dgamma)
                 self._give_grad(bn.bias, dbeta)
                 if conv.bias is not None:
@@ -396,7 +407,10 @@
                     if image._version != image_version:
                         raise RuntimeError("the network input was modified in place between forward and backward: the first "
                                            "convolution's weight gradient reads it (pass a copy, or finish backward first)")
-                    self._give_grad(conv.weight, ops.conv_first_wgrad(image, dy, out=self._dst(conv.weight)))
+                    if fold_first:
+                        self._give_grad(conv.weight, ops.conv_first_wgrad_bn(image, g0, y, vec, sums, out=self._dst(conv.weight)))
+                    else:
+                        self._give_grad(conv.weight, ops.conv_first_wgrad(image, dy, out=self._dst(conv.weight)))
                 elif im2col:
                     dwp = ops.wgrad(dy, x, (Cout, x.C), ntaps=1)
                     cin = conv.in_channels
@@ -1710,16 +1724,25 @@
         logits = ops.outconv_fwd(x, w, b, xform=xf)
         if self.record:
             def bwd(g_logits: torch.Tensor):
-                dx = self.new_act(x.N, x.H, x.W, x.C) if (x.needs_grad or xf is not None) else None
                 dwt = self._dst(conv.weight)
                 dbt = self._dst(conv.bias) if conv.bias is not None else None
                 src = getattr(x, "bn_src", None) if (sole_reader and (self.fuse_bn_reduce_convt or xf is not None)) else None
-                dw, db = ops.outconv_bwd(x, w, g_logits.contiguous().float(), dx,
-                                         dwt.view(K, x.C) if dwt is not None else None, dbt, bnred=src, lazy=xf is not None)
+                gl = g_logits.contiguous().float()
+                virt = (xf is not None and self.fold_head_grad and src is not None and self.training
+                        and not self.fuse_bn_finalize and ops.bn_bwd_head_supported(src[0], K))
+                dx = self.new_act(x.N, x.H, x.W, x.C) if ((x.needs_grad or xf is not None) and not virt) else None
+                if virt:
+                    dw, db, part = ops.outconv_bwd(x, w, gl, None, dwt.view(K, x.C) if dwt is not None else None, dbt,
+                                                   bnred=src, lazy=True, store_dx=False)
+                else:
+                    dw, db = ops.outconv_bwd(x, w, gl, dx, dwt.view(K, x.C) if dwt is not None else None, dbt, bnred=src,
+                                             lazy=xf is not None)
                 self._give_grad(conv.weight, dwt if dwt is not None else dw.reshape(conv.weight.shape))
                 if conv.bias is not None:
                     self._give_grad(conv.bias, db)
-                if dx is not None:
+                if virt:
+                    x.add_grad(ops.HeadGrad(gl, w, part))
+                elif dx is not None:
                     x.add_grad(dx)
 
             self._heads.append((bwd, 1))
diff --git a/unet_zoo_amd/ops.py b/unet_zoo_amd/ops.py
--- a/unet_zoo_amd/ops.py
+++ b/unet_zoo_amd/ops.py
@@ -247,6 +247,27 @@
     with _Timed("wgrad_first_bf16", 2.0 * N * H * W * 9 * C * Cout, 4.0 * x.numel() + 2.0 * dy.P * Cout):
         L.check(lib.uz_conv3x3_first_wgrad(L.dtype_code(dy.dtype), x.data_ptr(), N, C, H, W, dy.ptr(), dy.ld, Cout,
                                            out.data_ptr(), ws.data_ptr(), L.stream_ptr()), "uz_conv3x3_first_wgrad")
+    return out
+
+
+def conv_first_wgrad_bn(x: torch.Tensor, g: Act, y: Act, vec: torch.Tensor, sums: torch.Tensor,
+                        out: Optional[torch.Tensor] = None) -> torch.Tensor:
+    L.require_cuda(x, g.buf, y.buf)
+    N, C, H, W = x.shape
+    Cout = g.C
+    assert (y.N, y.H, y.W, y.C) == (g.N, g.H, g.W, g.C) == (N, H, W, Cout) and g.dtype == y.dtype == torch.bfloat16
+    assert sums.dtype == torch.float64 and sums.shape == (2, Cout) and sums.is_contiguous()
+    lib = L.load()
+    ws_bytes = L.check_count(lib.uz_conv3x3_first_wgrad_workspace_bytes(N, H, W, Cout), "uz_conv3x3_first_wgrad_workspace_bytes")
+    ws = torch.empty(ws_bytes // 4, dtype=torch.float32, device=x.device)
+    if out is None:
+        out = torch.empty((Cout, C, 3, 3), dtype=torch.float32, device=x.device)
+    assert out.numel() == Cout * C * 9 and out.is_contiguous() and out.dtype == torch.float32
+    with _Timed("wgrad_first_bf16", 2.0 * N * H * W * 9 * C * Cout, 4.0 * x.numel() + 4.0 * g.P * Cout):
+        L.check(lib.uz_conv3x3_first_wgrad_bn(L.dtype_code(g.dtype), x.data_ptr(), N, C, H, W, g.ptr(), g.ld, y.ptr(), y.ld,
+                                              vec[0].data_ptr(), vec[1].data_ptr(), vec[2].data_ptr(), vec[3].data_ptr(),
+                                              sums.data_ptr(), float(y.P), Cout, out.data_ptr(), ws.data_ptr(), L.stream_ptr()),
+                "uz_conv3x3_first_wgrad_bn")
     return out
 
 
@@ -499,15 +520,16 @@
 
 
 def bn_relu_bwd(y: Act, vec: torch.Tensor, g0: Optional[Act], g1: Optional[Act],
-                gpool: Optional[Act], sums: torch.Tensor, dy: Act, dgamma: torch.Tensor,
+                gpool: Optional[Act], sums: torch.Tensor, dy: Optional[Act], dgamma: torch.Tensor,
                 dbeta: torch.Tensor, pool_ceil: bool = False, relu: bool = True,
                 partials: Optional[torch.Tensor] = None, frozen: bool = False,
                 fin_flag: Optional[torch.Tensor] = None, reverse: bool = False) -> None:
     lib = L.load()
+    assert dy is not None or (fin_flag is None and not frozen)
     def desc(rev):
         return L.BnBwdDesc(L.dtype_code(y.dtype), y.N, y.H, y.W, y.C, y.ld,
                            g0.ld if g0 is not None else 0, g1.ld if g1 is not None else 0,
-                           gpool.ld if gpool is not None else 0, dy.ld,
+                           gpool.ld if gpool is not None else 0, dy.ld if dy is not None else 0,
                            int(pool_ceil) | (0 if relu else 2) | (4 if rev else 0))
     d = desc(reverse)
     d_apply = desc(reverse != (partials is None and BN_BWD_ALTERNATE))
@@ -544,11 +566,43 @@
         with _Timed("bn_relu_bwd_reduce", 0.0, es * y.P * y.C * (1 + nsrc)):
             L.check(lib.uz_bn_relu_bwd_reduce(byref(d), *args, ws.data_ptr(), sums.data_ptr(),
                                               dgamma.data_ptr(), dbeta.data_ptr(), s), "uz_bn_relu_bwd_reduce")
+    if dy is None:
+        return
     if frozen:
         sums.zero_()
     with _Timed("bn_relu_bwd_apply", 0.0, es * y.P * y.C * (2 + nsrc)):
         L.check(lib.uz_bn_relu_bwd_apply(byref(d_apply), *args, sums.data_ptr(), float(y.P), dy.ptr(), s),
                 "uz_bn_relu_bwd_apply")
+
+
+class HeadGrad:
+    __slots__ = ("g", "w", "bn_partials")
+
+    def __init__(self, g: torch.Tensor, w: torch.Tensor, bn_partials: torch.Tensor):
+        self.g, self.w, self.bn_partials = g, w, bn_partials
+
+
+def bn_bwd_head_supported(y: Act, K: int) -> bool:
+    return bool(L.load().uz_bn_relu_bwd_apply_head_supported(L.dtype_code(y.dtype), y.C, K)) and y.ld % 8 == 0
+
+
+def bn_relu_bwd_head(y: Act, vec: torch.Tensor, hg: HeadGrad, sums: torch.Tensor, dy: Act, dgamma: torch.Tensor,
+                     dbeta: torch.Tensor, reverse: bool = False) -> None:
+    lib = L.load()
+    K = hg.w.shape[0]
+    parts = hg.bn_partials
+    assert hg.g.dtype == torch.float32 and hg.g.is_contiguous() and hg.g.shape == (y.N, K, y.H, y.W)
+    assert hg.w.dtype == torch.float32 and hg.w.is_contiguous() and hg.w.shape == (K, y.C)
+    assert parts.shape[1:] == (2, y.C) and parts.is_contiguous() and bn_bwd_head_supported(y, K)
+    s = L.stream_ptr()
+    L.check(lib.uz_bn_bwd_finalize(parts.data_ptr(), parts.shape[0], y.C, sums.data_ptr(), dgamma.data_ptr(),
+                                   dbeta.data_ptr(), s), "uz_bn_bwd_finalize")
+    d = L.BnBwdDesc(L.dtype_code(y.dtype), y.N, y.H, y.W, y.C, y.ld, 0, 0, 0, dy.ld, 4 if reverse else 0)
+    es = y.buf.element_size()
+    with _Timed("bn_relu_bwd_apply_head", 2.0 * K * y.P * y.C, es * y.P * y.C * 2 + 4.0 * K * y.P):
+        L.check(lib.uz_bn_relu_bwd_apply_head(byref(d), y.ptr(), vec[0].data_ptr(), vec[1].data_ptr(), vec[2].data_ptr(),
+                                              vec[3].data_ptr(), hg.g.data_ptr(), hg.w.data_ptr(), K, sums.data_ptr(),
+                                              float(y.P), dy.ptr(), s), "uz_bn_relu_bwd_apply_head")
 
 
 def outconv_xform_supported(x: Act, K: int) -> bool:
@@ -573,7 +627,7 @@
 
 def outconv_bwd(x: Act, w: torch.Tensor, g: torch.Tensor, dx: Optional[Act],
                 dw: Optional[torch.Tensor] = None, db: Optional[torch.Tensor] = None,
-                bnred: Optional[tuple] = None, lazy: bool = False):
+                bnred: Optional[tuple] = None, lazy: bool = False, store_dx: bool = True):
     lib = L.load()
     K = w.shape[0]
     assert g.dtype == torch.float32 and g.is_contiguous() and g.shape == (x.N, K, x.H, x.W)
@@ -587,16 +641,20 @@
                         "uz_outconv_bwd_workspace_bytes")
     ws = torch.empty(wsb // 4, dtype=torch.float32, device=dev)
     if lazy:
-        assert bnred is not None and dx is not None and x.dtype == torch.bfloat16 and (bnred[0].P, bnred[0].C) == (x.P, x.C), \
+        assert bnred is not None and (dx is not None) == store_dx and x.dtype == torch.bfloat16 and (bnred[0].P, bnred[0].C) == (x.P, x.C), \
             "a head on a lazy activation takes its backward through uz_outconv_bwd_bnred"
-    if bnred is not None and dx is not None and x.dtype == torch.bfloat16 and (bnred[0].P, bnred[0].C) == (x.P, x.C):
+    assert store_dx or lazy
+    if bnred is not None and (dx is not None or not store_dx) and x.dtype == torch.bfloat16 and (bnred[0].P, bnred[0].C) == (x.P, x.C):
         bn_y, vec4 = bnred
         rows = L.check_count(lib.uz_outconv_bwd_rows(code, x.N, x.H * x.W, x.C), "uz_outconv_bwd_rows")
         part = torch.empty((rows, 2, x.C), dtype=torch.float32, device=dev)
         L.check(lib.uz_outconv_bwd_bnred(code, None if lazy else x.ptr(), x.ld, x.N, x.H * x.W, x.C, w.data_ptr(), K, g.data_ptr(),
-                                         dx.ptr(), dx.ld, dw.data_ptr(), db.data_ptr(), ws.data_ptr(), bn_y.ptr(), bn_y.ld,
+                                         dx.ptr() if store_dx else None, dx.ld if store_dx else 0, dw.data_ptr(), db.data_ptr(),
+                                         ws.data_ptr(), bn_y.ptr(), bn_y.ld,
                                          vec4[0].data_ptr(), vec4[1].data_ptr(), vec4[2].data_ptr(), vec4[3].data_ptr(),
                                          part.data_ptr(), L.stream_ptr()), "uz_outconv_bwd_bnred")
+        if not store_dx:
+            return dw.view(K, x.C), db, part
         dx.bn_partials = part
         return dw.view(K, x.C), db
     L.check(lib.uz_outconv_bwd(code, x.ptr(), x.ld, x.N, x.H * x.W, x.C, w.data_ptr(), K, g.data_ptr(),
```

Measured after the change: 2544 images/sec (median of 6 runs). 1.01x the previous value.
